# navigator8972/vae_assoc

Measured on AMD Instinct MI355X. Metric: paired-samples/sec (img+jnt assoc-VAE train step), higher is better.
Workload: dtype bf16

## Files before the change

### vae_assoc_amd/csrc/avae_device.h

```cpp
#pragma once
#include <hip/hip_runtime.h>
#include <math.h>
#include <stdint.h>
#include "../../include/avae.h"

namespace avae {

constexpr int kMaxMod = 4;
constexpr int kThreads = 256;
constexpr int kTileBytesK = 128;
constexpr int kRowAlign = 256;
constexpr int kLatentRows = 16;
constexpr int kAdamRows = 16;
constexpr int kCostHist = 4096;
constexpr int kSumsqThreads = 256;
constexpr int kSumsqMaxBlocks = 256;
constexpr int kSumsqQuads = 8;
inline int sumsq_blocks(long long p_int) {
    const long long quads = p_int / 4, per_block = (long long)kSumsqThreads * kSumsqQuads;
    const long long g = (quads + per_block - 1) / per_block;
    return (int)(g < 1 ? 1 : g > kSumsqMaxBlocks ? kSumsqMaxBlocks : g);
}
inline int sumsq_chain(long long p_int) {
    const long long quads = p_int / 4, per_pass = (long long)kSumsqThreads * sumsq_blocks(p_int);
// ... 20 lines not shown
    int lda, ldb;
    int tiles_m, tiles_n;
    int act;
    int ld0, ld1, ldx;
    int nz;
    int binary;
    int ksplit, kchunk;
    int bias_row;
    int bias_ep;
    int kin;
    int tile_off, tile_cnt;
    int slot_base;
    int n_slots;
    int n_mod;
    int bump_step;
    float scale;
    float lambda;
    float inv_bg;
    const void* A;
    const void* B;
    void* out0;
    void* out1;
    void* out2;
    const void* aux0;
    const void* aux1;
    const void* aux2;
    float* partial;
    const float* eps;
    float wts[kMaxMod];
    const void* tail_w;
    void* tail_out;
    const void* tail_aux;
    int tail_mode;
    int tail_n;
    int tail_ldw, tail_ldo, tail_ldx;
    int tail_act;
    int tail_kt;
    int conv;
    const unsigned char* present;
    int present_ld;
};

struct ConvA {
    const void* src;
    const void* consts;
    int M, K;
    int OHW, OW, IH, IW, Cin;
    int k, so, d, pad;
    int src_sb, src_sp;
    int ones;
    unsigned mg_ohw, mg_ow, mg_k, mg_cin;
};
constexpr int kMaxConvA = 12;
constexpr int kMaxItemsPerLaunch = 12;
constexpr int kMaxPf = 4;
struct LaunchArgs {
    int n_items;
    int grid_x;
    int sched;
    int n_pf;
    const void* pf_ptr[4];
    int pf_lines[4];
    const ConvA* conv_tab;
    WorkItem items[kMaxItemsPerLaunch];
};

struct TnItem {
    const void* A;
    const void* B;
    float* out;
    int M, N, K;
    int lda, ldb, ld0;
    int tiles_m, tiles_n;
    int ksplit, kchunk;
    int bias_row;
    int tile_off, tile_cnt;
    int conv;
    void* W; void* Wt;
    int ldw, ldt;
};
constexpr int kMaxTnItems = 32;
constexpr int kTnPieces = 8;
struct TnPiece { unsigned short item, tile_off, cum_end, pad; };
struct DevState;
struct TnLaunchArgs {
    int n_items;
    int grid_x;
    int xcd_group;
    int sched;
    int adam;
    long long d_theta, d_m, d_v;
    float beta1, beta2, eps;
    const DevState* st;
    const ConvA* conv_tab;
    int xcd_pieces;
    TnPiece pieces[8][kTnPieces];
    TnItem items[kMaxTnItems];
};
static_assert(sizeof(TnLaunchArgs) <= 4096, "kernel arguments are passed by value: 4 KiB");

struct DevState {
    long long step;
    float last_cost;
    float lr_t;
    float cost_hist[kCostHist];
};

struct ClipState {
    float max_norm;
    int skip_nonfinite;
    long long n_skipped;
    float partial[kSumsqMaxBlocks];
    float norm_hist[kCostHist];
};

struct EmaState {
    float decay;
    int warmup;
    int pad[30];
};
static_assert(sizeof(EmaState) == 128, "the average is line-aligned behind its settings");

struct HyperEntry { float kl, lambda, lr, pad; };
constexpr int kHyperSets = 16;
struct SchedState {
    avae_schedule sched[3];
    float lambda0, lr0;
    HyperEntry tab[kHyperSets];
    float hist[kCostHist][3];
};

__host__ __device__ inline float schedule_value(const avae_schedule& s, long long t) {
#pragma clang fp contract(off)
    long long u = t - 1;
    if (u < 0) u = 0;
    if (s.kind == AVAE_SCHED_PIECEWISE) {
        if (s.period > 0) u %= s.period;
        const int last = s.n_knots - 1;
        if (u <= s.knot_step[0]) return s.knot_value[0];
        if (u >= s.knot_step[last]) return s.knot_value[last];
        int i = 0;
        while (i + 1 < last && u >= s.knot_step[i + 1]) ++i;
        const double v0 = (double)s.knot_value[i], v1 = (double)s.knot_value[i + 1];
        const double f = (double)(u - s.knot_step[i]) / (double)(s.knot_step[i + 1] - s.knot_step[i]);
        return (float)(v0 + (v1 - v0) * f);
    }
    if (s.kind == AVAE_SCHED_EXP) {
        const double e = s.staircase ? (double)(u / s.decay_steps) : (double)u / (double)s.decay_steps;
        return (float)pow((double)s.decay_rate, e);
    }
    return 1.0f;
}

struct AdamItem {
    float* theta;
    float* m;
    float* v;
    const float* g;
    void* W;
    void* Wt;
    int rows, cols;
    int ld, ldt;
    int tiles_r, tiles_c, tile_base;
    int ldw;
    void* Wadj; void* Wf;
    int ldadj, ldf, adj_k, adj_cin;
};

constexpr int kMaxAdamItems = 80;
struct AdamArgs {
    const AdamItem* items;
    int n_items;
    int base[kMaxAdamItems];
    int mode;
    int book;
    float lr, beta1, beta2, eps;
    DevState* st;
    const float* cost_src;
    ClipState* clip;
    int n_partial;
    const EmaState* ema;
    float* avg;
// ... 155 lines not shown
    long long row0;
    unsigned long long seed; unsigned draw;
    const unsigned char* present; int pres_ld;
};
void launch_iw_latent(int compute_dtype, const IwLatentArgs& a, hipStream_t s);
struct IwRowsArgs {
    const float* xhat[kMaxMod]; int ldh[kMaxMod];
    const float* x[kMaxMod]; long long ldx[kMaxMod];
    int n_in[kMaxMod], binary[kMaxMod];
    float* ell;
    int n_dec, kc, n_mod;
    const unsigned char* present;
};
void launch_iw_rows(const IwRowsArgs& a, hipStream_t s);
struct IwReduceArgs {
    const float* ell; const float* r;
    float* state;
    float* out; int width;
    int rows, kc, src, n_mod;
    int first, last;
    float log_k;
    const unsigned char* present;
};
void launch_iw_reduce(const IwReduceArgs& a, hipStream_t s);

struct ImputeFuseArgs {
    const float* mulv[kMaxMod];
    unsigned mods;
    const unsigned char* present;
    float* fused;
    float* mu; float* lv;
    float* z32;
    void* Z[kMaxMod]; int ldz[kMaxMod]; int n_zdst;
    int rows, nz, n_mod;
};
void launch_impute_fuse(int compute_dtype, const ImputeFuseArgs& a, hipStream_t s);
struct ImputeAccumArgs {
    const float* xhat[kMaxMod]; int ldh[kMaxMod];
    float* mean[kMaxMod]; float* var[kMaxMod];
    int n_in[kMaxMod];
    int tile0[kMaxMod + 1];
    int col0[kMaxMod];
    float* state; int ld_state;
    int rows, kc, k0, K, n_mod;
};
void launch_impute_accum(const ImputeAccumArgs& a, hipStream_t s);

constexpr int kMaxWorld = 8;
constexpr int kIpcThreads = 256;
struct IpcArgs {
    float* g;
    long long off, granules;
    long long cost_idx;
    int world, rank, wire_bf16, blocks;
    unsigned char* peer[kMaxWorld];
    long long off_flag1, off_flag2;
    long long off_cost;
    long long off_seq;
    long long off_err;
    long long off_slots, slot_stride, off_res;
    unsigned long long timeout_ticks;
};
void launch_ipc_allreduce(const IpcArgs& a, hipStream_t s);
void launch_wire_pack(const float* g, void* wire, long long n, hipStream_t s);
void launch_wire_unpack(float* g, const void* wire, long long n, hipStream_t s);

struct LaunchEvents { hipEvent_t start, stop; };
extern thread_local LaunchEvents t_launch_events;

constexpr int kStampLaunches = 32, kStampBlocks = 1024, kStampWords = 8;

int tile_lds_bytes(int tile_cfg, bool two_c_tiles);
void launch_grouped(int compute_dtype, int tile_cfg, const LaunchArgs& args, int grid_x, int grid_y, int lds_bytes,
                    DevState* st, hipStream_t s, unsigned long long* stamps = nullptr, int launch_id = 0);
void launch_grouped_tn(int compute_dtype, int tile_cfg, const TnLaunchArgs& args, int grid_x, int grid_y, int lds_bytes,
                       DevState* st, hipStream_t s, unsigned long long* stamps = nullptr, int launch_id = 0);
void launch_adam(int compute_dtype, const AdamArgs& a, int n_blocks, hipStream_t s);
void launch_grad_sumsq(const float* g, long long p_int, float* partial, hipStream_t s);
void launch_prep(int compute_dtype, const PrepArgs& a, hipStream_t s);
const void* prep_kernel(int compute_dtype, bool masked, bool noisy, bool sched);
void launch_fill(void* base, int elem_bytes, unsigned bits, long long start, long long stride, int count, hipStream_t s);
void launch_sums(const ReduceArgs& a, int n_blocks, hipStream_t s);
int small_head_lds_bytes();
void launch_small_latb(int compute_dtype, int act, const LaunchArgs& args, int grid_x, int grid_y, int lds_bytes, DevState* st, hipStream_t s,
                       unsigned long long* stamps, int launch_id);
void launch_small_head(int compute_dtype, int act, const LaunchArgs& args, int grid_x, int grid_y, int lds_bytes, hipStream_t s,
                       unsigned long long* stamps, int launch_id);
void launch_small_tn(int compute_dtype, const TnLaunchArgs& args, int grid_x, int grid_y, hipStream_t s, unsigned long long* stamps, int launch_id);
void launch_small_loss(int compute_dtype, const LaunchArgs& args, int grid_x, int grid_y, int lds_bytes, hipStream_t s, unsigned long long* stamps, int launch_id);
void launch_small(int compute_dtype, const LaunchArgs& args, int grid_x, int grid_y, int lds_bytes, hipStream_t s, unsigned long long* stamps, int launch_id);
void launch_reduce(const ReduceArgs& a, int n_blocks, hipStream_t s);
void launch_chain2(int compute_dtype, const LaunchArgs& args, int grid_x, int grid_y, int lds_bytes, unsigned* counters, unsigned* err, hipStream_t s);

}
```

### vae_assoc_amd/csrc/avae_host.hip

```cpp
#include "avae_device.h"
#include "avae_complete.h"
#include "avae_retrieve.h"
#include "avae_latent_stats.h"
#include "../../include/avae.h"

#include <dlfcn.h>
#include <sched.h>
#include <unistd.h>

#include <algorithm>
#include <cctype>
#include <cstddef>
#include <cmath>
#include <cstdio>
#include <cstdlib>
#include <cstring>
#include <functional>
#include <map>
#include <mutex>
#include <stdexcept>
#include <string>
#include <vector>

using namespace avae;
// ... 110 lines not shown
    std::vector<ConvStage> cenc, cdec;
};

struct Launch {
    std::string name;
    int type = 0;
    int cfg = 0, first = 0, count = 0, blocks = 0, lds = 0;
    int lean_act = 0;
    int grid_x = 1, grid_y = 1;
    bool tn = false;
    LaunchArgs args{};
    TnLaunchArgs targs{};
    GatherArgs ga{};
    Col2imArgs ca{};
    ReduceArgs ra{};
    ThinArgs ta{};
    WadjArgs wa{};
    GpermArgs gp{};
    RowsumArgs rs{};
};

struct TimingRec { hipEvent_t a, b; int launch_name; };

struct StepGraph {
    hipGraphExec_t exec = nullptr;
    hipGraph_t graph = nullptr;
    hipGraphNode_t prep = nullptr;
    void release() {
        if (exec) (void)hipGraphExecDestroy(exec);
        if (graph) (void)hipGraphDestroy(graph);
        *this = StepGraph();
    }
};

struct StepPlan {
    std::vector<Launch> fwd;
    StepGraph full, multi[2], eval;
    void release() { full.release(); multi[0].release(); multi[1].release(); eval.release(); }
};

struct DevBuf {
    void* p = nullptr;
    size_t bytes = 0;
    DevBuf() = default;
    DevBuf(const DevBuf&) = delete;
    DevBuf& operator=(const DevBuf&) = delete;
    ~DevBuf() { if (p) (void)hipFree(p); }
    void* ensure(size_t n, bool zero = false) {
        if (p && n != bytes) throw Err("internal error: device scratch of " + std::to_string(bytes) + " bytes asked for as " + std::to_string(n));
        if (p) return p;
        void* q = nullptr;
        HIP_OK(hipMalloc(&q, n));
        if (zero && hipMemset(q, 0, n) != hipSuccess) { (void)hipFree(q); throw Err("hipMemset of fresh device scratch failed"); }
        p = q; bytes = n;
        return p;
    }
    template <typename T> T* as() const { return static_cast<T*>(p); }
};

}

struct avae_handle {
    avae_config cfg{};
    std::mutex mu;
    std::string err;
    int es = 2, KU = 64;
    int B = 0, Bp = 0, ldB = 0;
    int nz = 0, M = 0, ld_eps = 0;
    std::vector<Mod> mods;
    size_t P_flat = 0, P_int = 0, P_enc = 0;
    size_t off_theta = 0, off_m = 0, off_v = 0, off_g = 0;
    size_t stage_lo = 0, stage_bytes = 0;
    size_t off_eps = 0, off_partial = 0, off_state = 0, off_items = 0, off_adam = 0, off_inf = 0, off_stamps = 0, off_latent = 0;
    int n_partial = 0;
    size_t ws_bytes = 0;
    unsigned char* ws = nullptr;
    bool own_ws = false;
    hipStream_t cap_stream = nullptr;

    std::vector<WorkItem> items;
    std::vector<Launch> bwd;
    std::vector<Launch> wgrad;
    std::vector<Launch> wgrad_adam;
    int n_buckets = 1;
    int bwd_split = 0;
    std::vector<Launch> wgrad_b[2];
    struct Range { size_t off, count; };
    std::vector<Range> ranges_b[2];
    int adam_first_b[2] = {0, 0}, adam_count_b[2] = {0, 0}, adam_blocks_b[2] = {0, 0};
    std::vector<AdamItem> adam_items_b;
    size_t off_adam_b = 0;
    void* comm = nullptr;
    int comm_world = 1, comm_rank = 0;
    bool comm_on = false;
    size_t off_wire = 0;
    unsigned char* ipc_block = nullptr;
    size_t ipc_bytes = 0;
    unsigned char* ipc_peer[kMaxWorld] = {nullptr, nullptr, nullptr, nullptr, nullptr, nullptr, nullptr, nullptr};
    bool ipc_opened[kMaxWorld] = {false, false, false, false, false, false, false, false};
    bool ipc_attached = false;
    IpcArgs ipc_args{};
    hipStream_t comm_stream = nullptr;
    hipEvent_t ev_grad[2] = {nullptr, nullptr}, ev_red[2] = {nullptr, nullptr};
    std::vector<StepGraph> g_dp[2];
    StepGraph g_dpm[2];
    bool dp_graph_failed = false;
    Launch cost_only;
    std::vector<AdamItem> adam_items;
    int adam_blocks = 0;
    struct Inf { std::vector<WorkItem> items; std::vector<Launch> launches; int rows = -1; size_t dev_off = 0; };
    std::vector<Inf> inf_enc, inf_dec;
    struct Serve { int bucket = 0; std::vector<WorkItem> items; std::vector<Launch> launches; hipGraphExec_t graph = nullptr; ServeArgs in;
                   Launch in_launch; bool fused_in = false;
                   ServeInArgs in_lean; int in_lean_grid = 0; bool lean_in = false; };
    std::vector<Serve> serve;
    size_t off_slot = 0;
    DevBuf iw_buf;
    DevBuf imp_buf;
    DevBuf row_pres;
    DevBuf topk_buf;
    DevBuf stats_buf;
    size_t off_chain = 0;
    size_t off_consts = 0, off_conv_tab = 0;
    std::vector<ConvA> conv_tab;

    StepPlan plain, masked;
    DevBuf pres_buf;
    size_t pres_set = 0;

    avae_corruption corr{};
    unsigned drop_thr[kMaxMod] = {};

    bool clip_on = false;
    DevBuf clip_buf;
    long long clip_steps = 0;

    bool sched_on = false;
    DevBuf sched_buf;
    long long sched_steps = 0;

    bool ema_on = false, averaged = false;
    float ema_decay = 0.0f;
    int ema_warmup = 0;
    DevBuf ema_buf;

    struct Complete { bool built = false; std::vector<WorkItem> items; std::vector<Launch> fwd, bwd; CompleteArgs args{};
                      StepGraph g[3]; DevBuf buf; };
    Complete cmpl;

    hipStream_t last_stream = nullptr;
    bool has_last_stream = false;
    hipEvent_t ev_switch = nullptr;
    unsigned draw_id = 0;
    bool timing = false;
    bool debug_sync = false;
    std::vector<std::string> tnames;
    std::vector<TimingRec> trecs;

    template <typename T> T* at(size_t off) const { return reinterpret_cast<T*>(ws + off); }
    DevState* state() const { return at<DevState>(off_state); }
    float* grad() const { return at<float>(off_g); }
    float* ema_avg() const { return reinterpret_cast<float*>(ema_buf.as<unsigned char>() + sizeof(EmaState)); }
};

namespace {

inline int spread_ld(int ld, int KU, int es) {
    static const bool off = std::getenv("AVAE_NO_LD_SPREAD") != nullptr;
    return (!off && ((size_t)ld * es) % 512 == 0) ? ld + KU : ld;
}

Act make_act(Bump& b, int width, bool ones, int rows, int KU, int es, int ld = 0) {
    Act a;
    a.width = width;
    a.rows = rows;
    a.ones = ones;
    a.ld = ld > 0 ? ld : spread_ld((int)rup(width + 1, KU), KU, es);
    a.rm = b.take(rup(rows, kRowAlign) * (size_t)a.ld * es);
    return a;
}

Dense make_dense(Bump& b, size_t& pint, int in, int out, int KU, int es, bool head) {
    Dense d;
    d.in = in; d.out = out; d.head = head;
    d.ld = (int)rup(out, 32);
    d.ldw = spread_ld((int)rup(out, KU), KU, es);
    d.ldt = spread_ld((int)rup(in + 1, KU), KU, es);
    d.master = pint;
    pint += (size_t)(in + 1) * d.ld;
    d.W = b.take(rup(in + 1, kRowAlign) * (size_t)d.ldw * es);
    d.Wt = b.take(rup(out, kRowAlign) * (size_t)d.ldt * es);
    return d;
}

void check_config(const avae_config& c) {
    if (c.abi_version != AVAE_ABI_VERSION) throw Err("avae_config.abi_version mismatch");
    if (c.n_modalities < 1 || c.n_modalities > AVAE_MAX_MODALITIES) throw Err("n_modalities out of range");
    if (c.n_z < 1 || c.n_z > 64) throw Err("n_z must be in [1,64] (the fused head/latent epilogue holds 2*n_z columns in one tile)");
    if (c.batch_size < 1) throw Err("batch_size must be positive");
    if (c.compute_dtype != AVAE_F32 && c.compute_dtype != AVAE_BF16) throw Err("compute_dtype must be AVAE_F32 or AVAE_BF16");
    if (c.activation < AVAE_ACT_IDENTITY || c.activation > AVAE_ACT_TANH) throw Err("unknown activation");
    if (c.comm_buckets != 0 && c.comm_buckets != 1 && c.comm_buckets != 2) throw Err("comm_buckets must be 0, 1 or 2");
    if (c.wire_dtype != AVAE_F32 && c.wire_dtype != AVAE_BF16) throw Err("wire_dtype must be AVAE_F32 or AVAE_BF16");
    if (c.use_comm < AVAE_COMM_NONE || c.use_comm > AVAE_COMM_IPC) throw Err("use_comm must be AVAE_COMM_NONE, AVAE_COMM_RCCL or AVAE_COMM_IPC");
    for (int m = 0; m < c.n_modalities; ++m) {
        const avae_modality& mo = c.mod[m];
        if (mo.n_input < 1) throw Err("n_input must be positive");
        if (mo.hidden_conv) {
            if (mo.n_input != 784) throw Err("hidden_conv needs n_input = 784 (28x28 images)");
            if (!mo.binary) throw Err("hidden_conv needs a binary modality (the reference's non-binary conv decoder is shape-broken, vae_assoc.py:299)");
            if (mo.n_hidden_layers != 2 || mo.conv_gener[0] < 2 || mo.conv_gener[1] < 1) throw Err("hidden_conv needs n_hidden_recog_1/2 and n_hidden_gener_1 (>=2) / n_hidden_gener_2");
        }
        if (mo.n_hidden_layers < 1 || mo.n_hidden_layers > AVAE_MAX_HIDDEN) throw Err("n_hidden_layers out of range");
        for (int k = 0; k < mo.n_hidden_layers; ++k)
            if (mo.n_hidden[k] < 1) throw Err("hidden width must be positive");
    }
}

inline bool thin_fast(const ConvGeom& g) { return thin_fast_geometry(g) && !std::getenv("AVAE_NO_THIN_FAST"); }
inline int thin_split(const ConvGeom& g, int mode) {
    if (!thin_fast(g)) return kThinSplit;
    int sp[3] = {1, 4, 1};
    if (const char* e = std::getenv("AVAE_THIN_FAST_SPLIT")) std::sscanf(e, "%d,%d,%d", &sp[0], &sp[1], &sp[2]);
    const int v = sp[mode];
    return v == 1 || v == 2 || v == 4 ? v : 1;
}

void plan_memory(avae_handle* h) {
    const avae_config& c = h->cfg;
    h->es = c.compute_dtype == AVAE_BF16 ? 2 : 4;
    h->KU = kTileBytesK / h->es;
    h->B = c.batch_size;
    h->Bp = (int)rup(h->B, kRowAlign);
    h->ldB = (int)rup(h->B, h->KU);
    h->nz = c.n_z;
    h->ld_eps = (int)rup(c.n_z, 4);
    h->M = c.n_modalities;
    const int KU = h->KU, es = h->es, Bp = h->Bp, ldB = h->ldB, nz = h->nz, B = h->B;
// ... 638 lines not shown
    L.tn = true;
    for (int i = first; i < first + count; ++i) L.tn = L.tn && items[i].kind == K_WGRAD;
    if (count > (L.tn ? kMaxTnItems : kMaxItemsPerLaunch)) throw Err("internal error: too many items in one launch");
    std::memset(&L.args, 0, sizeof(L.args));
    std::memset(&L.targs, 0, sizeof(L.targs));
    if (L.tn) {
        int G = 1;
        if (L.cfg == 2) for (int g : {4, 2}) if (count % g == 0) { G = g; break; }
        if (const char* e = std::getenv("AVAE_TN_G")) G = std::atoi(e);
        if (G != 1 && G != 2 && G != 4 && G != 8) throw Err("AVAE_TN_G must be 1, 2, 4 or 8");
        auto tiles_of = [&](const WorkItem& w) { return w.tiles_m * w.tiles_n * (w.ksplit > 1 ? w.ksplit : 1); };
        int SX = L.grid_x;
        if (G == 1 && !std::getenv("AVAE_NO_TN_SLICES")) {
            long best = -1;
            for (int sx = 8; sx <= L.grid_x; sx += 8) {
                long entries = 0;
                for (int i = first; i < first + count; ++i) entries += (tiles_of(items[i]) + sx - 1) / sx;
                if (entries > kMaxTnItems) continue;
                if (best < 0 || entries * sx <= best) { best = entries * sx; SX = sx; }
            }
        }
        int n = 0;
        for (int i = 0; i < count; ++i) {
            const WorkItem& w = items[first + i];
            const int nt = tiles_of(w);
            for (int off = 0; off < nt; off += SX) {
                if (n >= kMaxTnItems) throw Err("internal error: too many weight-gradient entries");
                TnItem& t = L.targs.items[n++];
                t.A = w.A; t.B = w.B; t.out = reinterpret_cast<float*>(w.ksplit > 1 ? w.out1 : w.out0);
                t.bias_row = std::max(w.bias_row, 0);
                t.M = w.bias_row > 0 ? w.M - 1 : w.M; t.N = w.N; t.K = w.K; t.lda = w.lda; t.ldb = w.ldb; t.ld0 = w.ld0;
                t.tiles_m = w.tiles_m; t.tiles_n = w.tiles_n; t.ksplit = w.ksplit; t.kchunk = w.kchunk;
                t.tile_off = off; t.tile_cnt = std::min(SX, nt - off); t.conv = w.conv;
            }
        }
        if (G > 1 && !std::getenv("AVAE_NO_TN_BALANCE")) {
            std::vector<TnItem> ent(L.targs.items, L.targs.items + n);
            std::stable_sort(ent.begin(), ent.end(), [](const TnItem& a, const TnItem& b) { return a.tile_cnt > b.tile_cnt; });
            auto pack = [&](int g, std::vector<std::vector<TnItem>>& bins) {
                bins.assign(g, {});
                std::vector<long> load(g, 0);
                const int cap = kMaxTnItems / g;
                for (const TnItem& e : ent) {
                    int best = -1;
                    for (int p = 0; p < g; ++p) if ((int)bins[p].size() < cap && (best < 0 || load[p] < load[best])) best = p;
                    bins[best].push_back(e); load[best] += e.tile_cnt;
                }
                const long per_xcd = (*std::max_element(load.begin(), load.end()) * g + 7) / 8;
                return (per_xcd + 31) / 32;
            };
            std::vector<std::vector<TnItem>> bins, bins2;
            if (!std::getenv("AVAE_TN_G") && G == 4 && n * 2 <= kMaxTnItems * 2) {
                const long r4 = pack(4, bins), r2 = pack(2, bins2);
                if (r2 < r4) { G = 2; bins.swap(bins2); }
            } else {
                pack(G, bins);
            }
            size_t groups = 0;
            for (const auto& bn : bins) groups = std::max(groups, bn.size());
            std::memset(L.targs.items, 0, sizeof(L.targs.items));
            for (size_t g = 0; g < groups; ++g)
                for (int p = 0; p < G; ++p) if (g < bins[p].size()) L.targs.items[g * G + p] = bins[p][g];
            n = (int)groups * G;
        }
        L.grid_x = SX;
        L.targs.n_items = n;
        L.targs.grid_x = L.grid_x;
        L.targs.xcd_group = G;
        L.grid_y = (n + G - 1) / G * G;
        L.blocks = L.grid_x * L.grid_y;
    } else {
        L.args.n_items = count;
        L.args.grid_x = L.grid_x;
        for (int i = 0; i < count; ++i) L.args.items[i] = items[first + i];
    }
    L.args.conv_tab = L.targs.conv_tab = h->at<ConvA>(h->off_conv_tab);
    if (const char* e = std::getenv("AVAE_SCHED")) L.args.sched = L.targs.sched = std::atoi(e);
    if (*next_slot > h->n_partial) throw Err("internal error: cost partial slots overflow");
    return L;
}

void dp_ranges(const avae_handle* h, int* n_buckets, std::vector<avae_handle::Range> (&out)[2]);

void xcd_pieces(Launch& L) {
    TnLaunchArgs& a = L.targs;
    std::vector<TnItem> layers;
    for (int i = 0; i < a.n_items; ++i) {
        const TnItem& e = a.items[i];
        if (e.tile_cnt <= 0) continue;
        bool seen = false;
        for (const TnItem& l : layers) seen = seen || l.out == e.out;
        if (seen) continue;
        TnItem l = e;
        l.tile_off = 0; l.tile_cnt = e.tiles_m * e.tiles_n;
        if (l.tile_cnt > 65535) return;
        layers.push_back(l);
    }
    long total = 0;
    for (const TnItem& l : layers) total += l.tile_cnt;
    if (layers.empty() || total > 8L * 65535) return;
    const int quota = (int)((total + 7) / 8);
    std::vector<int> order(layers.size());
    for (size_t i = 0; i < order.size(); ++i) order[i] = (int)i;
    std::stable_sort(order.begin(), order.end(), [&](int x, int y) { return layers[x].tile_cnt > layers[y].tile_cnt; });
    struct Bin { int load = 0; std::vector<TnPiece> pc; };
    Bin bins[8];
    for (int li : order) {
        int off = 0, left = layers[li].tile_cnt;
        while (left > 0) {
            int best = -1;
            for (int b = 0; b < 8; ++b)
                if ((int)bins[b].pc.size() < kTnPieces && bins[b].load + left <= quota && (best < 0 || bins[b].load > bins[best].load)) best = b;
            int take = left;
            if (best < 0) {
                for (int b = 0; b < 8; ++b)
                    if ((int)bins[b].pc.size() < kTnPieces && bins[b].load < quota && (best < 0 || bins[b].load < bins[best].load)) best = b;
                if (best < 0) return;
                take = std::min(left, quota - bins[best].load);
            }
            bins[best].load += take;
            bins[best].pc.push_back(TnPiece{(unsigned short)li, (unsigned short)off, (unsigned short)bins[best].load, 0});
            off += take; left -= take;
        }
    }
    int longest = 0;
    for (int b = 0; b < 8; ++b) {
        longest = std::max(longest, bins[b].load);
        for (int i = 0; i < kTnPieces; ++i)
            a.pieces[b][i] = i < (int)bins[b].pc.size() ? bins[b].pc[i] : TnPiece{0, 0, (unsigned short)bins[b].load, 0};
    }
    std::memset(a.items, 0, sizeof(a.items));
    for (size_t i = 0; i < layers.size(); ++i) a.items[i] = layers[i];
    a.n_items = (int)layers.size();
    a.xcd_pieces = 1;
    L.grid_x = 8 * longest; L.grid_y = 1; L.blocks = L.grid_x;
    a.grid_x = L.grid_x;
}

struct Groups {
    avae_handle* h;
    std::vector<WorkItem>& items;
    int slot = 0;
    template <typename Fill> void operator()(const std::string& name, std::vector<Launch>& dst, Fill&& fill) {
        const int first = (int)items.size();
        fill();
        const int count = (int)items.size() - first;
        if (count > 0) dst.push_back(finish_launch(h, items, first, count, name, &slot));
    }
};

void build_training_plan(avae_handle* h) {
    h->items.clear(); h->plain.fwd.clear(); h->bwd.clear(); h->wgrad.clear(); h->conv_tab.clear();
    Builder bd(h, h->items, h->B, true);
    Groups group{h, h->items};
    int Lmax = 0;
    for (const Mod& md : h->mods) Lmax = std::max(Lmax, md.L);
    auto fuse_tail = [&](std::vector<Launch>& ls, int mode) {
        if (ls.size() < 2 || std::getenv("AVAE_NO_TAIL")) return false;
        Launch& Lp = ls[ls.size() - 2];
        Launch& Lc = ls[ls.size() - 1];
        if (Lp.type != 0 || Lc.type != 0 || Lp.tn || Lc.tn || Lp.cfg != 3) return false;
        const int want_p = mode == 1 ? K_FWD_HEAD : K_DGRAD_LATENT, want_c = mode == 1 ? K_FWD_HIDDEN : K_DGRAD_HIDDEN;
        std::vector<int> prod(Lc.count, -1);
        for (int i = 0; i < Lc.count; ++i) {
            const WorkItem& c = h->items[Lc.first + i];
            if (c.kind != want_c || c.bias_ep || c.K > 2 * h->KU || c.N > 1024) return false;
            for (int k = 0; k < Lp.count; ++k) {
                const WorkItem& n = h->items[Lp.first + k];
                if (n.kind != want_p || n.M != c.M) continue;
                const void* res = mode == 1 ? n.out1 : n.out0;
                const int ldres = mode == 1 ? n.ld1 : n.ld0;
                if (res && res == c.A && ldres == c.lda) prod[i] = k;
            }
            if (prod[i] < 0) return false;
        }
        for (int i = 0; i < Lc.count; ++i) {
            const WorkItem c = h->items[Lc.first + i];
            for (WorkItem* n : {&h->items[Lp.first + prod[i]], &Lp.args.items[prod[i]]}) {
                n->tail_mode = mode; n->tail_w = c.B; n->tail_ldw = c.ldb; n->tail_n = c.N; n->tail_out = c.out0; n->tail_ldo = c.ld0;
                n->tail_aux = c.aux0; n->tail_ldx = c.ldx; n->tail_act = c.act; n->tail_kt = c.K / h->KU;
                n->tiles_n = (c.N + 63) / 64;
            }
        }
        int max_tiles = 1;
        for (int k = 0; k < Lp.count; ++k) max_tiles = std::max(max_tiles, h->items[Lp.first + k].tiles_m * h->items[Lp.first + k].tiles_n);
        Lp.grid_x = (max_tiles + 7) & ~7; Lp.blocks = Lp.grid_x * Lp.grid_y; Lp.args.grid_x = Lp.grid_x;
        Lp.name += "+" + Lc.name;
        ls.pop_back();
        if (!std::getenv("AVAE_NO_LEAN") && !std::getenv("AVAE_NO_LEAN_HEAD")) {
            bool lean = true;
            int act = -1;
            for (int k = 0; k < Lp.count; ++k) {
                const WorkItem& n = h->items[Lp.first + k];
                if (n.kind == K_COST) continue;
                lean = lean && n.kind == want_p && n.tail_mode == mode
                            && (act < 0 || act == n.tail_act) && n.K > 0 && 2 * n.nz <= 64 && n.tail_kt >= 1 && n.tail_kt <= 2;
                act = n.tail_act;
            }
            if (lean && mode == 1)
                for (int k = 0; k < Lp.count; ++k) lean = lean && h->items[Lp.first + k].kind == K_FWD_HEAD && h->items[Lp.first + k].out1 != nullptr;
            if (lean) { Lp.cfg = mode == 2 ? 10 : 11; Lp.lds = small_head_lds_bytes(); Lp.lean_act = act; }
        }
        return true;
    };
    auto every_conv = [](const Mod&) { return true; };
    auto gather_launch = [&](const std::string& name, std::vector<Launch>& dst, auto&& stage_of, auto&& src_of, auto&& want) {
        Launch L;
        L.name = name; L.type = 1;
        int base = 0;
        for (Mod& md : h->mods) if (md.conv && want(md)) {
            GatherSeg g = bd.gather_seg(stage_of(md), src_of(md));
            g.tile_base = base; base += g.tiles_r * g.tiles_c;
            L.ga.seg[L.ga.n_seg++] = g;
        }
        L.blocks = base;
        if (base > 0) dst.push_back(L);
    };
    auto col2im_launch = [&](const std::string& name, std::vector<Launch>& dst, auto&& stage_of, auto&& prev_of, auto&& want) {
        Launch L;
        L.name = name; L.type = 2;
        int base = 0;
        for (Mod& md : h->mods) if (md.conv && want(md)) {
            Col2imSeg c = bd.col2im_seg(stage_of(md), prev_of(md), md);
            c.tile_base = base; base += c.tiles_r * c.tiles_c;
            L.ca.seg[L.ca.n_seg++] = c;
        }
        L.blocks = base;
        if (base > 0) dst.push_back(L);
    };
    auto thin_launch = [&](const std::string& name, std::vector<Launch>& dst, int mode, int i) {
        Launch L;
        L.name = name; L.type = 4;
        L.ta.mode = mode;
        int base = 0;
        for (Mod& md : h->mods) if (md.conv && md.cdec[i].thin) {
            ThinSeg t = bd.thin_seg(md.cdec[i], md.cdec[i - 1]);
            t.split = thin_split(md.cdec[i].g, mode);
            t.block_base = base;
            base += h->B * t.split;
            L.ta.seg[L.ta.n_seg++] = t;
        }
        L.blocks = base;
        if (base > 0) dst.push_back(L);
    };
    auto is_adj = [&](int i) { bool t = false; for (const Mod& md : h->mods) t = t || (md.conv && i >= 0 && i <= 3 && md.cdec[i].adj); return t; };
    auto is_thin = [&](int i) { bool t = false; for (const Mod& md : h->mods) t = t || (md.conv && md.cdec[i].thin); return t; };
    bool any_conv = false;
    for (const Mod& md : h->mods) any_conv = any_conv || md.conv;
    for (int k = 0; k < Lmax; ++k)
        group("fwd_enc" + std::to_string(k + 1), h->plain.fwd, [&] {
            for (Mod& md : h->mods) if (k < md.L) h->items.push_back(bd.fwd_hidden(k == 0 ? md.X0 : md.E[k - 1], md.enc[k], md.E[k]));
        });
    if (std::getenv("AVAE_CHAIN2") && !any_conv && h->plain.fwd.size() == 2 && h->plain.fwd[0].cfg == 7 && h->plain.fwd[1].cfg == 7 && h->plain.fwd[0].count == h->plain.fwd[1].count
        && 2 * h->plain.fwd[0].count <= kMaxItemsPerLaunch) {
        Launch& A = h->plain.fwd[0];
        const Launch& Bn = h->plain.fwd[1];
        bool ok = true;
        for (int i = 0; i < A.count; ++i) {
            const WorkItem& a = A.args.items[i];
            const WorkItem& c = Bn.args.items[i];
            ok = ok && a.kind == K_FWD_HIDDEN && c.kind == K_FWD_HIDDEN && a.act == c.act && a.M == c.M && a.N == c.N && a.tiles_m == c.tiles_m && a.tiles_n == c.tiles_n
                    && c.A == a.out0 && c.lda == a.ld0 && a.N % 4 == 0 && a.tiles_m <= 64;
        }
        if (ok) {
            for (int i = 0; i < A.count; ++i) A.args.items[A.count + i] = Bn.args.items[i];
            A.args.n_items = 2 * A.count;
            A.cfg = 13; A.name += "+" + Bn.name;
            h->plain.fwd.pop_back();
        }
    }
    if (any_conv) {
        for (int i = 0; i < 3; ++i) {
            auto src_of = [&, i](Mod& md) { return i == 0 ? h->at<void>(md.X0.rm) : h->at<void>(md.cenc[i - 1].Y.rm); };
            gather_launch("conv_enc" + std::to_string(i + 1) + "_im2col", h->plain.fwd, [&](Mod& md) -> const ConvStage& { return md.cenc[i]; },
                          src_of, [i](const Mod& md) { return !md.cenc[i].impl; });
            group("conv_enc" + std::to_string(i + 1), h->plain.fwd, [&] {
                for (Mod& md : h->mods) if (md.conv) h->items.push_back(md.cenc[i].impl ? bd.conv_fwd_impl(md.cenc[i], src_of(md)) : bd.conv_fwd(md.cenc[i])); });
        }
        gather_launch("conv_head_im2col", h->plain.fwd, [&](Mod& md) -> const ConvStage& { return md.cenc[3]; },
                      [&](Mod& md) { return h->at<void>(md.cenc[2].Y.rm); }, [](const Mod& md) { return !md.cenc[3].impl; });
    }
    group("fwd_head", h->plain.fwd, [&] { for (Mod& md : h->mods) h->items.push_back(bd.fwd_head(md, true, md.conv && md.cenc[3].impl)); });
    bool latent_alone = false;
    {
// ... 307 lines not shown
                for (int k = md.L - 1; k >= 1; --k) set[0].push_back(bd.wgrad(md.D[k - 1], md.dec[k], md.dD[k]));
                set[0].push_back(bd.wgrad(md.Z, md.dec[0], md.dD[0]));
                set[1].push_back(bd.wgrad(md.E.back(), md.head, md.dH));
                for (int k = md.L - 1; k >= 1; --k) set[1].push_back(bd.wgrad(md.E[k - 1], md.enc[k], md.dE[k]));
                set[1].push_back(bd.wgrad(md.X0, md.enc[0], md.dE[0]));
            }
            wgrad_launches(set[0], h->wgrad_b[0], "wgrad_dec");
            wgrad_launches(set[1], h->wgrad_b[1], "wgrad_enc");
        }
        for (int i = 1; i <= 3; ++i) if (is_thin(i)) thin_launch("conv_dec" + std::to_string(i + 1) + "_wgrad_direct", h->wgrad, 2, i);
        {
            Launch L;
            L.name = "conv_bias_rowsum"; L.type = 8;
            int base = 0;
            for (Mod& md : h->mods) if (md.conv) for (const ConvStage& st : md.cdec) if (st.adj && !st.impl_w) {
                RowsumSeg& g = L.rs.seg[L.rs.n_seg++];
                g.src = h->at<void>(st.dY.rm); g.part = h->at<float>(st.rs_part); g.ld = st.dY.ld;
                g.rows = h->B * st.g.OH * st.g.OW; g.cols = st.d.out; g.cols4 = st.rs_cols4; g.n_blocks = kRowsumBlocks;
                g.cpow = 4; while (g.cpow < g.cols4) g.cpow *= 2;
                if (g.cpow > 64) throw Err("internal error: bias row sums hold at most 64 columns");
                g.block_base = base; base += kRowsumBlocks;
            }
            L.blocks = base;
            if (base > 0) h->wgrad.push_back(L);
        }
        {
            Launch R;
            R.name = "conv_wgrad_sums"; R.type = 5;
            int base = 0;
            for (Mod& md : h->mods) if (md.conv) for (const ConvStage& st : md.cdec) if (st.adj && !st.impl_w) {
                ReduceSeg& g = R.ra.seg[R.ra.n_seg++];
                g.dst = h->grad() + st.d.master + (size_t)st.d.in * st.d.ld; g.src = h->at<float>(st.rs_part);
                g.n = st.d.out; g.parts = kRowsumBlocks; g.stride = st.rs_cols4; g.dst_ld = 1;
                g.block_base = base; base += (g.n + 3) / 4;
            }
            for (Mod& md : h->mods) if (md.conv) for (const ConvStage& st : md.cdec) if (st.thin) {
                ReduceSeg& g = R.ra.seg[R.ra.n_seg++];
                g.dst = h->grad() + st.d.master; g.src = h->at<float>(st.thin_part);
                g.n = st.d.in + 1; g.parts = st.thin_blocks; g.stride = st.thin_kp; g.dst_ld = st.d.ld;
                g.block_base = base; base += (g.n + 3) / 4;
            }
            R.blocks = base;
            for (int i = 0; i < R.ra.n_seg; ++i) { R.ra.seg[i].colsum = 1; R.ra.seg[i].perm_k = 0; }
            if (base > 0) h->wgrad.push_back(R);
        }
        {
            Launch R;
            R.name = "wgrad_reduce"; R.type = 3;
            int base = 0;
            Launch* prev = (!h->wgrad.empty() && h->wgrad.back().type == 5 && !std::getenv("AVAE_NO_SUMS_MERGE")) ? &h->wgrad.back() : nullptr;
            if (prev) { R = *prev; R.name = prev->name + "+wgrad_reduce"; R.type = 9; base = prev->blocks; }
            for (const WorkItem& w : wg) if (w.ksplit > 1) {
                if (R.ra.n_seg >= kMaxReduceSegs) throw Err("internal error: too many split weight gradients");
                ReduceSeg& g = R.ra.seg[R.ra.n_seg++];
                g.dst = reinterpret_cast<float*>(w.out0); g.src = reinterpret_cast<const float*>(w.out1);
                g.n = w.M * w.ld0; g.parts = w.ksplit; g.stride = (long long)w.M * w.ld0;
                g.colsum = 0; g.perm_k = 0;
                if (!std::getenv("AVAE_NO_SUMS_MERGE"))
                    for (Mod& md : h->mods) if (md.conv) for (const ConvStage& st : md.cdec) if (st.adj && st.aksplit > 1 && g.dst == h->at<float>(st.Gadj)) {
                        g.dst = h->grad() + st.d.master;
                        g.perm_k = st.g.k; g.perm_cin = st.g.Cin; g.perm_cout = st.d.out; g.perm_ldga = st.ldga; g.perm_ld = st.d.ld;
                    }
                g.block_base = base; base += (g.n / 4 + kThreads - 1) / kThreads;
            }
            R.blocks = base;
            if (prev && base > prev->blocks) *prev = R;
            else if (!prev && base > 0) h->wgrad.push_back(R);
        }
        {
            Launch L;
            L.name = "conv_wgrad_perm"; L.type = 7;
            int base = 0;
            for (Mod& md : h->mods) if (md.conv) for (const ConvStage& st : md.cdec) if (st.adj && !st.impl_w) {
                if (st.aksplit > 1 && !std::getenv("AVAE_NO_SUMS_MERGE")) continue;
                GpermSeg& g = L.gp.seg[L.gp.n_seg++];
                g.Gadj = h->at<float>(st.Gadj); g.G = h->grad() + st.d.master; g.ldga = st.ldga; g.ld = st.d.ld;
                g.k = st.g.k; g.Cin = st.g.Cin; g.Cout = st.d.out;
                g.block_base = base; base += (st.g.Cin * st.g.k * st.g.k * st.d.out + kThreads - 1) / kThreads;
            }
            L.blocks = base;
            if (base > 0) h->wgrad.push_back(L);
        }
    }
    h->wgrad_adam.clear();
    if (!any_conv && h->wgrad.size() == 1 && h->wgrad[0].tn && h->wgrad[0].cfg == 0 && h->wgrad[0].targs.xcd_group == 1
        && !std::getenv("AVAE_NO_LEAN") && !std::getenv("AVAE_NO_ADAM_FUSE")) {
        Launch L = h->wgrad[0];
        bool ok = true;
        for (int i = 0; i < L.targs.n_items && ok; ++i) {
            TnItem& t = L.targs.items[i];
            ok = t.ksplit <= 1 && t.bias_row == 0 && t.K > 0;
            const Dense* dm = nullptr;
            for (const Mod& md : h->mods) {
                auto look = [&](const Dense& d) { if (h->grad() + d.master == t.out) dm = &d; };
                for (const Dense& d : md.enc) look(d);
                look(md.head);
                for (const Dense& d : md.dec) look(d);
                look(md.outl);
            }
            ok = ok && dm && t.M == dm->in + 1 && t.N == dm->out && t.ld0 == dm->ld;
            if (ok) { t.W = h->at<void>(dm->W); t.Wt = h->at<void>(dm->Wt); t.ldw = dm->ldw; t.ldt = dm->ldt; }
        }
        if (ok) {
            L.cfg = 12; L.name = "wgrad+adam";
            L.targs.adam = 1;
            L.targs.d_theta = h->at<float>(h->off_theta) - h->grad();
            L.targs.d_m = h->at<float>(h->off_m) - h->grad();
            L.targs.d_v = h->at<float>(h->off_v) - h->grad();
            L.targs.beta1 = h->cfg.beta1; L.targs.beta2 = h->cfg.beta2; L.targs.eps = h->cfg.adam_eps;
            L.targs.st = h->state();
            if (!std::getenv("AVAE_NO_XCD_PIECES")) xcd_pieces(L);
            h->wgrad_adam.push_back(L);
        }
    }
    if (!std::getenv("AVAE_NO_WARM")) {
        std::vector<Launch*> seq;
        for (Launch& L : h->plain.fwd) seq.push_back(&L);
        for (Launch& L : h->bwd) seq.push_back(&L);
        for (size_t i = 0; i < seq.size(); ++i) {
            Launch& L = *seq[i];
            if (L.type != 0 || L.tn || (L.cfg != 2 && L.cfg != 6)) continue;
            for (size_t j = i + 1; j < seq.size(); ++j) {
                const Launch& Nx = *seq[j];
                if (Nx.type != 0) continue;
                if (Nx.tn) break;
                for (int k = 0; k < Nx.args.n_items && L.args.n_pf < kMaxPf; ++k) {
                    const WorkItem& w = Nx.args.items[k];
                    if (!is_gemm(w.kind) || w.kind == K_WGRAD) continue;
                    const long bytes = (long)w.N * w.ldb * h->es;
                    if (bytes < 128 * 1024) continue;
                    L.args.pf_ptr[L.args.n_pf] = w.B; L.args.pf_lines[L.args.n_pf] = (int)(bytes / 128); ++L.args.n_pf;
                }
                break;
            }
        }
    }
    {
        const int first = (int)h->items.size();
        h->items.push_back(bd.cost(false));
        h->cost_only = finish_launch(h, h->items, first, 1, "cost_reduce", &group.slot);
    }

    h->adam_items.clear();
    int base = 0;
    auto add = [&](const Dense& d) {
        AdamItem a;
        std::memset(&a, 0, sizeof(a));
        a.theta = h->at<float>(h->off_theta) + d.master;
        a.m = h->at<float>(h->off_m) + d.master;
        a.v = h->at<float>(h->off_v) + d.master;
        a.g = h->grad() + d.master;
        a.W = h->at<void>(d.W); a.Wt = h->at<void>(d.Wt);
        a.rows = d.in + 1; a.cols = d.out; a.ld = d.ld; a.ldw = d.ldw; a.ldt = d.ldt;
        a.tiles_r = (a.rows + kAdamRows - 1) / kAdamRows; a.tiles_c = (a.cols + 63) / 64; a.tile_base = base;
        base += a.tiles_r * a.tiles_c;
        h->adam_items.push_back(a);
    };
    for (const Mod& md : h->mods) {
        if (md.conv) {
            for (const std::vector<ConvStage>* side : {&md.cenc, &md.cdec})
                for (const ConvStage& st : *side) {
                    add(st.d);
                    if ((st.adj && !std::getenv("AVAE_NO_WADJ_FOLD")) || st.impl_bwd) {
                        AdamItem& a = h->adam_items.back();
                        a.Wadj = h->at<void>(st.Wadj); a.ldadj = st.ldadj; a.adj_k = st.g.k; a.adj_cin = st.g.Cin;
                        if (st.adj) { a.Wf = h->at<void>(st.Wf); a.ldf = st.ldf; }
                    }
                }
            continue;
        }
        for (const Dense& d : md.enc) add(d);
        add(md.head);
        for (const Dense& d : md.dec) add(d);
        add(md.outl);
    }
    h->adam_blocks = base;
    h->adam_items_b.clear();
    for (int bk = 0; bk < 2; ++bk) {
        h->adam_first_b[bk] = (int)h->adam_items_b.size();
        int tb = 0;
        size_t i = 0;
        for (const Mod& md : h->mods) {
            const size_t n_enc = md.conv ? md.cenc.size() : (size_t)md.L + 1, n_all = md.conv ? md.cenc.size() + md.cdec.size() : 2 * (size_t)md.L + 2;
            for (size_t k = 0; k < n_all; ++k) {
                const int which = h->n_buckets == 1 ? 0 : (k < n_enc ? 1 : 0);
                if (which == bk) {
                    AdamItem a = h->adam_items[i + k];
                    a.tile_base = tb; tb += a.tiles_r * a.tiles_c;
                    h->adam_items_b.push_back(a);
                }
            }
            i += n_all;
        }
        h->adam_count_b[bk] = (int)h->adam_items_b.size() - h->adam_first_b[bk];
        h->adam_blocks_b[bk] = tb;
// ... 21 lines not shown
        inf.launches.push_back(L);
    };
    if (enc && md.conv) {
        for (int i = 0; i < 3; ++i) {
            gather1(md.cenc[i], i == 0 ? h->at<void>(md.X0.rm) : h->at<void>(md.cenc[i - 1].Y.rm), "inf_conv_im2col");
            one(bd.conv_fwd(md.cenc[i]), "inf_conv_enc");
        }
        gather1(md.cenc[3], h->at<void>(md.cenc[2].Y.rm), "inf_conv_im2col");
        one(bd.fwd_head(md, true), "inf_head");
    } else if (enc) {
        for (int k = 0; k < md.L; ++k) one(bd.fwd_hidden(k == 0 ? md.X0 : md.E[k - 1], md.enc[k], md.E[k]), "inf_enc");
        one(bd.fwd_head(md, true), "inf_head");
    } else if (md.conv) {
        for (int i = 0; i < 4; ++i) {
            if (md.cdec[i].dense_map) {
                Launch L;
                L.name = "inf_conv_dec_direct"; L.type = 4;
                L.ta.mode = 0;
                ThinSeg t = bd.thin_seg(md.cdec[i], md.cdec[i - 1]);
                t.block_base = 0;
                L.ta.seg[0] = t; L.ta.n_seg = 1;
                L.blocks = rows * t.split;
                inf.launches.push_back(L);
                continue;
            }
            gather1(md.cdec[i], i == 0 ? h->at<void>(md.Z.rm) : h->at<void>(md.cdec[i - 1].Y.rm), "inf_conv_im2col");
            one(bd.conv_fwd(md.cdec[i]), "inf_conv_dec");
        }
        if (!md.cdec[3].dense_map) gather1(md.cdec[4], h->at<void>(md.cdec[3].Y.rm), "inf_conv_im2col");
        one(bd.fwd_out(md, m, false), "inf_out");
    } else {
        for (int k = 0; k < md.L; ++k) one(bd.fwd_hidden(k == 0 ? md.Z : md.D[k - 1], md.dec[k], md.D[k]), "inf_dec");
        one(bd.fwd_out(md, m, false), "inf_out");
    }
    inf.rows = rows;
}

int tname_id(avae_handle* h, const std::string& n) {
    for (size_t i = 0; i < h->tnames.size(); ++i) if (h->tnames[i] == n) return (int)i;
    h->tnames.push_back(n);
    return (int)h->tnames.size() - 1;
}

struct Timed {
    avae_handle* h; hipStream_t s; bool on; hipEvent_t a = nullptr, b = nullptr; int id = 0;
    Timed(avae_handle* h_, hipStream_t s_, const std::string& name) : h(h_), s(s_), on(h_->timing && h_->trecs.size() < 200000) {
        if (!on) return;
        id = tname_id(h, name);
        HIP_OK(hipEventCreate(&a)); HIP_OK(hipEventCreate(&b));
        t_launch_events = LaunchEvents{a, b};
    }
    ~Timed() {
        if (!on) return;
        if (t_launch_events.start) {
            t_launch_events = LaunchEvents{nullptr, nullptr};
            (void)hipEventRecord(a, s); (void)hipEventRecord(b, s);
        }
        h->trecs.push_back(TimingRec{a, b, id});
    }
};

template <typename F> void timed_launch(avae_handle* h, hipStream_t s, const char* name, F&& launch) {
    Timed t(h, s, name);
    launch();
    LAUNCH_OK(name);
}

Launch relocated(const avae_handle* h, const Launch& L0, int j, const HyperEntry* hyper = nullptr) {
    Launch L = L0;
    const unsigned char* lo = h->ws + h->stage_lo;
    const unsigned char* hi = lo + h->stage_bytes;
    const size_t delta = (size_t)j * h->stage_bytes;
    auto fix = [&](auto& ptr) {
        const unsigned char* q = reinterpret_cast<const unsigned char*>(ptr);
        if (q >= lo && q < hi) ptr = reinterpret_cast<std::remove_reference_t<decltype(ptr)>>(const_cast<unsigned char*>(q) + delta);
    };
    for (int i = 0; i < L.args.n_items && L.type == 0; ++i) {
        WorkItem& w = L.args.items[i];
        fix(w.A); fix(w.B); fix(w.out0); fix(w.out1); fix(w.out2); fix(w.aux0); fix(w.aux1); fix(w.aux2); fix(w.eps);
        fix(w.tail_w); fix(w.tail_out); fix(w.tail_aux);
        if (w.present) w.present += (size_t)j * h->pres_set;
        if (hyper && (w.kind == K_LATENT || (w.kind == K_COST && w.bump_step))) w.tail_w = hyper + j;
    }
    for (int i = 0; i < L.targs.n_items && L.type == 0; ++i) { TnItem& t = L.targs.items[i]; fix(t.A); fix(t.B); fix(t.out); }
    for (int i = 0; i < L.ga.n_seg && L.type == 1; ++i) fix(L.ga.seg[i].src);
    return L;
}

void run_launch(avae_handle* h, const Launch& L, hipStream_t s, unsigned long long* stamps, int stamp) {
    Timed t(h, s, L.name);
    if (L.type == 1) launch_gather(h->cfg.compute_dtype, L.ga, L.blocks, s);
    else if (L.type == 2) launch_col2im(h->cfg.compute_dtype, L.ca, L.blocks, s);
    else if (L.type == 3) launch_reduce(L.ra, L.blocks, s);
    else if (L.type == 4) launch_thin(h->cfg.compute_dtype, L.ta, L.blocks, s);
    else if (L.type == 5) launch_colsum(L.ra, L.blocks, s);
    else if (L.type == 6) launch_wadj(h->cfg.compute_dtype, L.wa, L.blocks, s);
    else if (L.type == 7) launch_gperm(L.gp, L.blocks, s);
    else if (L.type == 8) launch_rowsum(h->cfg.compute_dtype, L.rs, L.blocks, s);
    else if (L.type == 9) launch_sums(L.ra, L.blocks, s);
    else if (L.cfg == 13) launch_chain2(h->cfg.compute_dtype, L.args, L.grid_x, L.grid_y, L.lds, h->at<unsigned>(h->off_chain), h->at<unsigned>(h->off_chain) + kMaxMod * 64, s);
    else if (L.cfg == 11) launch_small_head(h->cfg.compute_dtype, L.lean_act, L.args, L.grid_x, L.grid_y, L.lds, s, stamps, stamp);
    else if (L.cfg == 10) launch_small_latb(h->cfg.compute_dtype, L.lean_act, L.args, L.grid_x, L.grid_y, L.lds, h->state(), s, stamps, stamp);
    else if (L.cfg == 9) launch_small_loss(h->cfg.compute_dtype, L.args, L.grid_x, L.grid_y, L.lds, s, stamps, stamp);
    else if (L.cfg == 7) launch_small(h->cfg.compute_dtype, L.args, L.grid_x, L.grid_y, L.lds, s, stamps, stamp);
    else if (L.tn && L.cfg == 12) launch_small_tn(h->cfg.compute_dtype, L.targs, L.grid_x, L.grid_y, s, stamps, stamp);
    else if (L.tn) launch_grouped_tn(h->cfg.compute_dtype, L.cfg, L.targs, L.grid_x, L.grid_y, L.lds, h->state(), s, stamps, stamp);
    else launch_grouped(h->cfg.compute_dtype, L.cfg, L.args, L.grid_x, L.grid_y, L.lds, h->state(), s, stamps, stamp);
    LAUNCH_OK(L.name);
    if (h->debug_sync) {
        std::fprintf(stderr, "[avae] launch %s type=%d cfg=%d items=%d blocks=%d\n", L.name.c_str(), L.type, L.cfg, L.count, L.blocks);
        for (int i = 0; i < L.args.n_items && L.type == 0; ++i)
            std::fprintf(stderr, "        item kind=%d M=%d N=%d K=%d lda=%d ldb=%d tiles=%dx%d\n", L.args.items[i].kind, L.args.items[i].M,
                         L.args.items[i].N, L.args.items[i].K, L.args.items[i].lda, L.args.items[i].ldb, L.args.items[i].tiles_m, L.args.items[i].tiles_n);
        for (int i = 0; i < L.ga.n_seg && L.type == 1; ++i)
            std::fprintf(stderr, "        gather B=%d IH=%d Cin=%d OH=%d k=%d so=%d d=%d pad=%d sb=%d sp=%d ones=%d ldp=%d tiles=%dx%d\n", L.ga.seg[i].g.B, L.ga.seg[i].g.IH,
                         L.ga.seg[i].g.Cin, L.ga.seg[i].g.OH, L.ga.seg[i].g.k, L.ga.seg[i].g.so, L.ga.seg[i].g.d, L.ga.seg[i].g.pad, L.ga.seg[i].g.src_sb, L.ga.seg[i].g.src_sp,
                         L.ga.seg[i].g.ones, L.ga.seg[i].ldp, L.ga.seg[i].tiles_r, L.ga.seg[i].tiles_c);
        for (int i = 0; i < L.ca.n_seg && L.type == 2; ++i)
            std::fprintf(stderr, "        col2im B=%d IH=%d Cin=%d OH=%d k=%d lddp=%d lda=%d g0=%p tiles=%dx%d\n", L.ca.seg[i].g.B, L.ca.seg[i].g.IH, L.ca.seg[i].g.Cin,
                         L.ca.seg[i].g.OH, L.ca.seg[i].g.k, L.ca.seg[i].lddp, L.ca.seg[i].lda, (const void*)L.ca.seg[i].g0, L.ca.seg[i].tiles_r, L.ca.seg[i].tiles_c);
        std::fflush(stderr);
        HIP_OK(hipStreamSynchronize(s));
    }
}

bool has_hyper_item(const Launch& L) {
    for (int i = 0; i < L.args.n_items && L.type == 0; ++i)
        if (L.args.items[i].kind == K_LATENT || (L.args.items[i].kind == K_COST && L.args.items[i].bump_step)) return true;
    return false;
}

void run_set(avae_handle* h, const std::vector<Launch>& ls, size_t lo, size_t hi, int j, hipStream_t s, int stamp_base = -1, bool train = false) {
    unsigned long long* stamps = nullptr;
#ifdef AVAE_STAMPS
    if (stamp_base >= 0) stamps = h->at<unsigned long long>(h->off_stamps);
#endif
    const HyperEntry* hyper = nullptr;
    if (train && h->sched_on) {
        if (!h->sched_buf.p) throw Err("internal error: a schedule is on without its device state");
        if (j < 0 || j >= kHyperSets) throw Err("internal error: staging set outside the schedule table");
        hyper = h->sched_buf.as<SchedState>()->tab;
    }
    for (size_t i = lo; i < hi && i < ls.size(); ++i) {
        const int k = stamp_base + (int)(i - lo);
        if (j == 0 && !(hyper && has_hyper_item(ls[i]))) run_launch(h, ls[i], s, stamps, k);
        else run_launch(h, relocated(h, ls[i], j, hyper), s, stamps, k);
    }
}

void run_launches(avae_handle* h, const std::vector<Launch>& ls, hipStream_t s) { run_set(h, ls, 0, ls.size(), 0, s); }

void run_adam(avae_handle* h, int mode, hipStream_t s, int bucket = -1, bool from_avg = false) {
    AdamArgs a;
    std::memset(&a, 0, sizeof(a));
    int blocks = h->adam_blocks;
    if (bucket < 0) {
        a.items = h->at<AdamItem>(h->off_adam);
        a.n_items = (int)h->adam_items.size();
        if (a.n_items > kMaxAdamItems) throw Err("internal error: too many Adam items");
        for (int i = 0; i < a.n_items; ++i) a.base[i] = h->adam_items[i].tile_base;
    } else {
        a.items = h->at<AdamItem>(h->off_adam_b) + h->adam_first_b[bucket];
        a.n_items = h->adam_count_b[bucket];
        for (int i = 0; i < a.n_items; ++i) a.base[i] = h->adam_items_b[h->adam_first_b[bucket] + i].tile_base;
        blocks = h->adam_blocks_b[bucket];
        if (blocks == 0) return;
    }
    a.book = (bucket <= 0) ? 1 : 0;
    a.mode = mode;
    a.lr = h->cfg.learning_rate; a.beta1 = h->cfg.beta1; a.beta2 = h->cfg.beta2; a.eps = h->cfg.adam_eps;
    a.st = h->state();
    a.cost_src = h->grad() + h->P_int;
    a.clip = (mode == 0 && h->clip_on) ? h->clip_buf.as<ClipState>() : nullptr;
    a.n_partial = sumsq_blocks((long long)h->P_int);
    if (mode == 0 ? h->ema_on : from_avg) {
        if (!h->ema_buf.p) throw Err("internal error: averaging is on without its device state");
        a.ema = h->ema_buf.as<EmaState>(); a.avg = h->ema_avg(); a.theta0 = h->at<float>(h->off_theta);
    }
    Timed t(h, s, mode == 0 ? (bucket < 0 ? "adam" : bucket == 0 ? "adam_dec" : "adam_enc") : "shadow_refresh");
    launch_adam(h->cfg.compute_dtype, a, blocks, s);
    LAUNCH_OK(mode == 0 ? "adam" : "shadow_refresh");
}

void run_grad_sumsq(avae_handle* h, hipStream_t s) {
    ClipState* cs = h->clip_buf.as<ClipState>();
    if (!cs) throw Err("internal error: clipping is on without its device state");
    timed_launch(h, s, "grad_sumsq", [&] { launch_grad_sumsq(h->grad(), (long long)h->P_int, cs->partial, s); });
}

struct PrepIn { const float* const* in = nullptr; const int32_t* in_ld = nullptr; bool corrupt = false; };

PrepArgs new_prep(const avae_handle* h, unsigned long long salt, int row0 = 0) {
    PrepArgs a;
// ... 36 lines not shown
    fill_prep_eps(h, a, eps, rows);
    a.n_steps = n_steps; a.blocks_per_step = a.total_tiles + a.eps_blocks; a.set_stride = (long long)h->stage_bytes;
    if (present) { a.pres_src = present; a.pres_dst = h->pres_buf.as<unsigned char>(); a.pres_ld = h->M; }
    if (h->sched_on && salt == kTrainSalt) a.sched = h->sched_buf.as<SchedState>();
    return a;
}

void run_prep_batch(avae_handle* h, const float* const* x, const int32_t* x_ld, const float* eps, int rows,
                    unsigned long long salt, hipStream_t s, const uint8_t* present = nullptr, int n_steps = 1, const PrepIn& pin = PrepIn()) {
    const PrepArgs a = make_prep_batch(h, x, x_ld, eps, rows, salt, n_steps, present, pin);
    timed_launch(h, s, "prep", [&] { launch_prep(h->cfg.compute_dtype, a, s); });
}

struct PrepOne {
    const float* src; int src_ld, rows, cols;
    const Act& dst;
    int row0;
    PrepOne(const float* src_, int src_ld_, int rows_, int cols_, const Act& dst_, int row0_ = 0)
        : src(src_), src_ld(src_ld_), rows(rows_), cols(cols_), dst(dst_), row0(row0_) {}
    float* dst32 = nullptr; int ld32 = 0;
    bool eps = false;
    const float* eps_src = nullptr;
    unsigned long long salt = 0;
    PrepOne& with_eps(const float* e, unsigned long long salt_ = 0) { eps = true; eps_src = e; salt = salt_; return *this; }
    const unsigned char* pres_src = nullptr; unsigned char* pres_dst = nullptr; int pres_ld = 0;
};

void run_prep_single(avae_handle* h, const PrepOne& p, hipStream_t s) {
    PrepArgs a = new_prep(h, p.salt, p.row0);
    if (p.pres_src) { a.pres_src = p.pres_src; a.pres_dst = p.pres_dst; a.pres_ld = p.pres_ld; }
    if (p.src || p.pres_src) {
        a.n_seg = 1;
        a.total_tiles = fill_prep_seg(h, a.seg[0], p.src, p.src_ld, p.rows, p.cols, p.dst, p.dst32, p.ld32, 0);
    }
    if (p.eps) fill_prep_eps(h, a, p.eps_src, p.rows);
    launch_prep(h->cfg.compute_dtype, a, s);
    LAUNCH_OK("prep");
}

StepGraph capture(avae_handle* h, const std::function<void(hipStream_t)>& body, bool with_prep = false) {
    StepGraph sg;
    const bool tsave = h->timing;
    h->timing = false;
    HIP_OK(hipStreamBeginCapture(h->cap_stream, hipStreamCaptureModeThreadLocal));
    try { body(h->cap_stream); }
    catch (...) { (void)hipStreamEndCapture(h->cap_stream, &sg.graph); sg.release(); h->timing = tsave; throw; }
    h->timing = tsave;
    HIP_OK(hipStreamEndCapture(h->cap_stream, &sg.graph));
    try {
        if (with_prep) {
            size_t n_root = 0;
            HIP_OK(hipGraphGetRootNodes(sg.graph, nullptr, &n_root));
            if (n_root != 1) throw Err("internal error: the captured step is not a chain");
            HIP_OK(hipGraphGetRootNodes(sg.graph, &sg.prep, &n_root));
            hipGraphNodeType ty;
            HIP_OK(hipGraphNodeGetType(sg.prep, &ty));
            if (ty != hipGraphNodeTypeKernel) throw Err("internal error: the captured step does not start with the staging kernel");
        }
        HIP_OK(hipGraphInstantiate(&sg.exec, sg.graph, nullptr, nullptr, 0));
        if (!with_prep) { HIP_OK(hipGraphDestroy(sg.graph)); sg.graph = nullptr; }
    } catch (...) { sg.release(); throw; }
    return sg;
}

void patch_prep(avae_handle* h, const StepGraph& sg, const float* const* x, const int32_t* x_ld, const float* eps,
                int n_steps, const uint8_t* present, const PrepIn& pin) {
    PrepArgs a = make_prep_batch(h, x, x_ld, eps, h->B, kTrainSalt, n_steps, present, pin);
    void* kp[1] = {&a};
    hipKernelNodeParams np;
    std::memset(&np, 0, sizeof(np));
    np.func = const_cast<void*>(prep_kernel(h->cfg.compute_dtype, present != nullptr, a.noisy != 0, a.sched != nullptr));
    np.gridDim = dim3((a.total_tiles + a.eps_blocks) * n_steps); np.blockDim = dim3(kThreads);
    np.sharedMemBytes = 0; np.kernelParams = kp; np.extra = nullptr;
    HIP_OK(hipGraphExecKernelNodeSetParams(sg.exec, sg.prep, &np));
}

void fill_ones(avae_handle* h, const Act& a, hipStream_t s) {
    if (!a.ones) return;
    const unsigned bits = h->es == 2 ? 0x3F80u : 0x3F800000u;
    launch_fill(h->at<void>(a.rm), h->es, bits, a.width, a.ld, h->B, s);
    LAUNCH_OK("fill");
}

void step_body(avae_handle* h, const std::vector<Launch>& fwd, hipStream_t s, int j, int stamp_base = -1) {
    auto sb = [&](size_t k) { return stamp_base < 0 ? -1 : stamp_base + (int)k; };
    run_set(h, fwd, 0, fwd.size(), j, s, stamp_base, true);
    run_set(h, h->bwd, 0, h->bwd.size(), j, s, sb(fwd.size()), true);
    if (!h->wgrad_adam.empty() && !h->clip_on && !h->ema_on) {
        run_set(h, h->wgrad_adam, 0, h->wgrad_adam.size(), j, s, sb(fwd.size() + h->bwd.size()), true);
        return;
    }
    run_set(h, h->wgrad, 0, h->wgrad.size(), j, s, sb(fwd.size() + h->bwd.size()), true);
    if (h->clip_on) run_grad_sumsq(h, s);
    run_adam(h, 0, s);
}

void capture_steps(avae_handle* h, StepPlan& p, const uint8_t* present) {
    std::vector<const float*> x0(h->M, h->at<float>(h->mods[0].X32));
    try {
        p.full = capture(h, [&](hipStream_t cs) {
            run_prep_batch(h, x0.data(), nullptr, nullptr, h->B, kTrainSalt, cs, present);
            step_body(h, p.fwd, cs, 0, 0);
        }, true);
        for (int gi = 0; gi < 2; ++gi) p.multi[gi] = capture(h, [&](hipStream_t cs) {
            run_prep_batch(h, x0.data(), nullptr, nullptr, h->B, kTrainSalt, cs, present, kMultiSizes[gi]);
            for (int j = 0; j < kMultiSizes[gi]; ++j) step_body(h, p.fwd, cs, j);
        }, true);
    } catch (...) { p.full.release(); p.multi[0].release(); p.multi[1].release(); throw; }
}

void capture_plan(avae_handle* h, StepPlan& p, const uint8_t* present) {
    try {
        capture_steps(h, p, present);
        p.eval = capture(h, [&](hipStream_t cs) { run_launches(h, p.fwd, cs); run_launch(h, h->cost_only, cs, nullptr, -1); });
    } catch (...) { p.release(); throw; }
}

void init_device(avae_handle* h) {
    hipStream_t s = h->cap_stream;
    HIP_OK(hipMemsetAsync(h->ws, 0, h->ws_bytes, s));
    for (const Mod& md : h->mods) {
        for (int j = 0; j < kMultiSteps; ++j) {
            Act x = md.X0;
            x.rm += (size_t)j * h->stage_bytes;
            fill_ones(h, x, s);
        }
        for (const Act& a : md.E) fill_ones(h, a, s);
        fill_ones(h, md.Z, s);
        for (const Act& a : md.D) fill_ones(h, a, s);
        if (md.conv && md.cdec[3].dense_map) fill_ones(h, md.cdec[3].Y, s);
    }
    build_training_plan(h);
    HIP_OK(hipMemcpyAsync(h->at<void>(h->off_adam), h->adam_items.data(), h->adam_items.size() * sizeof(AdamItem), hipMemcpyHostToDevice, s));
    HIP_OK(hipMemcpyAsync(h->at<void>(h->off_adam_b), h->adam_items_b.data(), h->adam_items_b.size() * sizeof(AdamItem), hipMemcpyHostToDevice, s));
    {
        static const unsigned char c32_bf16[32] = {0, 0, 0, 0, 0, 0, 0, 0, 0, 0, 0, 0, 0, 0, 0, 0, 0x80, 0x3F};
        static const unsigned char c32_f32[32] = {0, 0, 0, 0, 0, 0, 0, 0, 0, 0, 0, 0, 0, 0, 0, 0, 0, 0, 0x80, 0x3F};
        HIP_OK(hipMemcpyAsync(h->at<void>(h->off_consts), h->es == 2 ? c32_bf16 : c32_f32, 32, hipMemcpyHostToDevice, s));
        if (!h->conv_tab.empty()) {
            const unsigned char* lo = h->ws + h->stage_lo;
            for (const ConvA& c : h->conv_tab)
                if (reinterpret_cast<const unsigned char*>(c.src) >= lo && reinterpret_cast<const unsigned char*>(c.src) < lo + h->stage_bytes * kMultiSteps)
                    throw Err("internal error: an implicit patch matrix on a staged input (not relocatable per step)");
            HIP_OK(hipMemcpyAsync(h->at<void>(h->off_conv_tab), h->conv_tab.data(), h->conv_tab.size() * sizeof(ConvA), hipMemcpyHostToDevice, s));
        }
    }
    size_t off = h->off_inf;
    h->inf_enc.assign(h->M, avae_handle::Inf());
    h->inf_dec.assign(h->M, avae_handle::Inf());
    for (int m = 0; m < h->M; ++m) {
        h->inf_enc[m].dev_off = off; off += ((size_t)h->mods[m].L + 1) * sizeof(WorkItem);
        h->inf_dec[m].dev_off = off; off += ((size_t)h->mods[m].L + 1) * sizeof(WorkItem);
    }
    HIP_OK(hipStreamSynchronize(s));
    if (h->cfg.use_graph) capture_plan(h, h->plain, nullptr);
}

void comm_check_error(avae_handle* h);

void fetch_cost(avae_handle* h, float* cost_host, bool from_state, hipStream_t s) {
    if (!cost_host) return;
    const void* src = from_state ? (const void*)&h->state()->last_cost : (const void*)(h->grad() + h->P_int);
    HIP_OK(hipMemcpyAsync(cost_host, src, sizeof(float), hipMemcpyDeviceToHost, s));
    HIP_OK(hipStreamSynchronize(s));
    comm_check_error(h);
}

void copy_rows(void* dst, size_t dpitch, const void* src, size_t spitch, size_t width, size_t rows, hipStream_t s) {
    HIP_OK(hipMemcpy2DAsync(dst, dpitch, src, spitch, width, rows, hipMemcpyDeviceToDevice, s));
}

hipStream_t on_stream(avae_handle* h, void* stream) {
    hipStream_t s = reinterpret_cast<hipStream_t>(stream);
    if (h->has_last_stream && s != h->last_stream) {
        if (!h->ev_switch) HIP_OK(hipEventCreateWithFlags(&h->ev_switch, hipEventDisableTiming));
        if (hipEventRecord(h->ev_switch, h->last_stream) == hipSuccess) HIP_OK(hipStreamWaitEvent(s, h->ev_switch, 0));
        else (void)hipGetLastError();
    }
    h->last_stream = s; h->has_last_stream = true;
    return s;
}

void check_schedule(const avae_schedule& c, const std::string& who) {
    auto fail = [&](const std::string& what) { throw Err(who + ": " + what); };
    if (c.kind == AVAE_SCHED_NONE) return;
    if (c.kind == AVAE_SCHED_PIECEWISE) {
        if (c.n_knots < 1 || c.n_knots > AVAE_SCHED_MAX_KNOTS)
            fail("n_knots = " + std::to_string(c.n_knots) + " must be in [1, " + std::to_string(AVAE_SCHED_MAX_KNOTS) + "]");
        if (c.period < 0) fail("period = " + std::to_string((long long)c.period) + " must be >= 0");
// ... 734 lines not shown
    HIP_OK(hipDeviceSynchronize());
    run_adam(h, 1, nullptr, -1, on);
    HIP_OK(hipDeviceSynchronize());
    h->averaged = on;
}

void set_ema(avae_handle* h, float decay, int32_t warmup) {
    if (!(decay >= 0.0f && decay < 1.0f)) throw Err("avae_set_ema: decay must be in (0, 1), or 0 to switch averaging off");
    if (warmup != 0 && warmup != 1) throw Err("avae_set_ema: warmup must be 0 or 1");
    const bool on = decay > 0.0f;
    HIP_OK(hipDeviceSynchronize());
    if (!on && !h->ema_buf.p) return;
    if (!on && h->averaged) use_averaged(h, false);
    h->ema_buf.ensure(sizeof(EmaState) + h->P_int * sizeof(float));
    if (on) {
        EmaState v;
        std::memset(&v, 0, sizeof(v));
        v.decay = decay; v.warmup = warmup;
        HIP_OK(hipMemcpy(h->ema_buf.p, &v, sizeof(v), hipMemcpyHostToDevice));
        h->ema_decay = decay; h->ema_warmup = warmup;
    }
    if (on == h->ema_on && (!h->cfg.use_graph || h->plain.full.exec)) return;
    if (on && !h->ema_on) ema_from_theta(h);
    h->plain.full.release(); h->plain.multi[0].release(); h->plain.multi[1].release();
    h->masked.full.release(); h->masked.multi[0].release(); h->masked.multi[1].release();
    for (StepGraph& g : h->g_dpm) g.release();
    h->ema_on = on;
    if (h->cfg.use_graph) {
        capture_steps(h, h->plain, nullptr);
        if (!h->masked.fwd.empty()) capture_steps(h, h->masked, h->pres_buf.as<unsigned char>());
    }
}

void destroy_handle(avae_handle* h) {
    int prev_dev = -1;
    if (hipGetDevice(&prev_dev) != hipSuccess) prev_dev = -1;
    (void)hipSetDevice(h->cfg.device);
    (void)hipDeviceSynchronize();
    h->plain.release();
    h->masked.release();
    for (StepGraph& g : h->g_dpm) g.release();
    for (std::vector<StepGraph>& v : h->g_dp) for (StepGraph& g : v) g.release();
    for (avae_handle::Serve& sv : h->serve) if (sv.graph) (void)hipGraphExecDestroy(sv.graph);
    for (StepGraph& g : h->cmpl.g) g.release();
    if (h->ev_switch) (void)hipEventDestroy(h->ev_switch);
    if (h->comm) { try { (void)Rccl::get().destroy(h->comm); } catch (...) {} }
    for (int r = 0; r < kMaxWorld; ++r) if (h->ipc_opened[r] && h->ipc_peer[r]) (void)hipIpcCloseMemHandle(h->ipc_peer[r]);
    if (h->ipc_block) (void)hipFree(h->ipc_block);
    for (int b = 0; b < 2; ++b) { if (h->ev_grad[b]) (void)hipEventDestroy(h->ev_grad[b]); if (h->ev_red[b]) (void)hipEventDestroy(h->ev_red[b]); }
    if (h->comm_stream) (void)hipStreamDestroy(h->comm_stream);
    for (TimingRec& r : h->trecs) { (void)hipEventDestroy(r.a); (void)hipEventDestroy(r.b); }
    if (h->cap_stream) (void)hipStreamDestroy(h->cap_stream);
    if (h->own_ws && h->ws) (void)hipFree(h->ws);
    const int dev = h->cfg.device;
    delete h;
    if (prev_dev >= 0 && prev_dev != dev) (void)hipSetDevice(prev_dev);
}

}

extern "C" {

int avae_workspace_bytes(const avae_config* cfg, size_t* bytes) {
    try {
        if (!cfg || !bytes) throw Err("null argument");
        check_config(*cfg);
        avae_handle tmp;
        tmp.cfg = *cfg;
        plan_memory(&tmp);
        *bytes = tmp.ws_bytes;
        return 0;
    } catch (const std::exception& e) { g_create_error = e.what(); return 2; }
}

int avae_create(const avae_config* cfg, avae_handle** out) {
    avae_handle* h = nullptr;
    try {
        if (!cfg || !out) throw Err("null argument");
        check_config(*cfg);
        h = new avae_handle();
        h->cfg = *cfg;
        if (const char* e = std::getenv("AVAE_DEBUG_SYNC")) h->debug_sync = e[0] == '1';
        if (h->debug_sync) h->cfg.use_graph = 0;
        if (h->cfg.beta1 == 0.f && h->cfg.beta2 == 0.f && h->cfg.adam_eps == 0.f) { h->cfg.beta1 = 0.9f; h->cfg.beta2 = 0.999f; h->cfg.adam_eps = 1e-8f; }
        int ndev = 0;
        HIP_OK(hipGetDeviceCount(&ndev));
        if (ndev < 1) throw Err("no HIP device: libavae has no CPU fallback");
        if (h->cfg.device < 0 || h->cfg.device >= ndev) throw Err("device ordinal out of range");
        DeviceGuard dg(h->cfg.device);
        hipDeviceProp_t prop;
        HIP_OK(hipGetDeviceProperties(&prop, h->cfg.device));
        if (std::string(prop.gcnArchName).rfind("gfx950", 0) != 0)
            throw Err(std::string("libavae is built for gfx950 only; device is ") + prop.gcnArchName);
        plan_memory(h);
        if (cfg->workspace) {
            if (cfg->workspace_bytes < h->ws_bytes) throw Err("workspace too small");
            if (reinterpret_cast<uintptr_t>(cfg->workspace) % 256) throw Err("workspace must be 256-byte aligned");
            h->ws = reinterpret_cast<unsigned char*>(cfg->workspace);
        } else {
            HIP_OK(hipMalloc(reinterpret_cast<void**>(&h->ws), h->ws_bytes));
            h->own_ws = true;
        }
        HIP_OK(hipStreamCreateWithFlags(&h->cap_stream, hipStreamNonBlocking));
        init_device(h);
        if (h->cfg.use_comm) comm_init(h);
        *out = h;
        return 0;
    } catch (const std::exception& e) {
        g_create_error = e.what();
        if (h) destroy_handle(h);
        return 2;
    }
}

void avae_destroy(avae_handle* h) {
    if (h) destroy_handle(h);
}

const char* avae_last_error(const avae_handle* h) { return h ? h->err.c_str() : g_create_error.c_str(); }

int avae_param_count(const avae_handle* h, size_t* n) {
    if (!h || !n) return 1;
    *n = h->P_flat;
    return 0;
}

int avae_get_params(avae_handle* h, float* host_dst) {
    return guarded(h, [&] { std::vector<float> I; master_to_host(h, h->off_theta, I); convert_params<false>(h, host_dst, I.data()); });
}

int avae_set_params(avae_handle* h, const float* host_src) {
    return guarded(h, [&] {
        std::vector<float> I(h->P_int, 0.0f);
        convert_params<true>(h, const_cast<float*>(host_src), I.data());
        host_to_master(h, h->off_theta, I);
        run_adam(h, 1, nullptr);
        HIP_OK(hipDeviceSynchronize());
        h->averaged = false;
    });
}

int avae_get_grads(avae_handle* h, float* host_dst) {
    return guarded(h, [&] { std::vector<float> I; master_to_host(h, h->off_g, I); convert_params<false>(h, host_dst, I.data()); });
}

int avae_get_opt_state(avae_handle* h, float* host_m, float* host_v, int64_t* step) {
    return guarded(h, [&] {
        std::vector<float> I;
        if (host_m) { master_to_host(h, h->off_m, I); convert_params<false>(h, host_m, I.data()); }
        if (host_v) { master_to_host(h, h->off_v, I); convert_params<false>(h, host_v, I.data()); }
        if (step) { long long st = 0; HIP_OK(hipDeviceSynchronize()); HIP_OK(hipMemcpy(&st, &h->state()->step, sizeof(st), hipMemcpyDeviceToHost)); *step = st; }
    });
}

int avae_set_opt_state(avae_handle* h, const float* host_m, const float* host_v, int64_t step) {
    return guarded(h, [&] {
        std::vector<float> I(h->P_int, 0.0f);
        if (host_m) { convert_params<true>(h, const_cast<float*>(host_m), I.data()); host_to_master(h, h->off_m, I); }
        if (host_v) { std::fill(I.begin(), I.end(), 0.0f); convert_params<true>(h, const_cast<float*>(host_v), I.data()); host_to_master(h, h->off_v, I); }
        long long st = step;
        HIP_OK(hipDeviceSynchronize());
        HIP_OK(hipMemcpy(&h->state()->step, &st, sizeof(st), hipMemcpyHostToDevice));
    });
}

int avae_stage_batches_in(avae_handle* h, int32_t n_steps, const float* const* x_dev, const int32_t* x_ld, const float* const* in_dev,
// ... 860 lines not shown
            }
            uint64_t P = 0;
            if (std::fread(&P, 8, 1, f) != 1 || P != h->P_flat) throw Err("checkpoint parameter count mismatch");
            if (std::fread(&st, 8, 1, f) != 1) throw Err("truncated checkpoint");
            th.resize(P); mm.resize(P); vv.resize(P);
            if (std::fread(th.data(), 4, P, f) != P || std::fread(mm.data(), 4, P, f) != P || std::fread(vv.data(), 4, P, f) != P)
                throw Err("truncated checkpoint");
            if (version == 3) {
                if (std::fread(&decay, 4, 1, f) != 1) throw Err("truncated checkpoint");
                warmup = r32();
                if (!(decay > 0.0f && decay < 1.0f) || warmup > 1) throw Err("checkpoint holds invalid averaging settings");
                av.resize(P);
                if (std::fread(av.data(), 4, P, f) != P) throw Err("truncated checkpoint");
            }
        } catch (...) { std::fclose(f); throw; }
        std::fclose(f);
        std::vector<float> I(h->P_int, 0.0f);
        convert_params<true>(h, th.data(), I.data()); host_to_master(h, h->off_theta, I);
        std::fill(I.begin(), I.end(), 0.0f); convert_params<true>(h, mm.data(), I.data()); host_to_master(h, h->off_m, I);
        std::fill(I.begin(), I.end(), 0.0f); convert_params<true>(h, vv.data(), I.data()); host_to_master(h, h->off_v, I);
        long long step = st;
        HIP_OK(hipMemcpy(&h->state()->step, &step, sizeof(step), hipMemcpyHostToDevice));
        run_adam(h, 1, nullptr);
        HIP_OK(hipDeviceSynchronize());
        h->averaged = false;
        if (version == 3) {
            set_ema(h, decay, (int32_t)warmup);
            std::fill(I.begin(), I.end(), 0.0f); convert_params<true>(h, av.data(), I.data()); host_to_ema(h, I);
        } else if (h->ema_on) {
            ema_from_theta(h);
        }
    });
}

int avae_synchronize(avae_handle* h) {
    return guarded(h, [&] { HIP_OK(hipDeviceSynchronize()); comm_check_error(h); });
}

int avae_timing_enable(avae_handle* h, int32_t on) {
    return guarded(h, [&] {
        HIP_OK(hipDeviceSynchronize());
        for (TimingRec& r : h->trecs) { (void)hipEventDestroy(r.a); (void)hipEventDestroy(r.b); }
        h->trecs.clear();
        h->timing = on != 0;
    });
}

int avae_timing_report(avae_handle* h, char* buf, size_t buf_bytes) {
    return guarded(h, [&] {
        HIP_OK(hipDeviceSynchronize());
        const double cal_ms = 0.0;
        std::vector<double> sum(h->tnames.size(), 0.0), mn(h->tnames.size(), 1e30);
        std::vector<long> cnt(h->tnames.size(), 0);
        for (TimingRec& r : h->trecs) {
            float ms = 0.f;
            HIP_OK(hipEventElapsedTime(&ms, r.a, r.b));
            sum[r.launch_name] += ms; cnt[r.launch_name] += 1; mn[r.launch_name] = std::min(mn[r.launch_name], (double)ms);
        }
        std::string out;
        for (size_t i = 0; i < h->tnames.size(); ++i) {
            if (!cnt[i]) continue;
            char line[256];
            std::snprintf(line, sizeof(line), "%s %ld %.6f %.6f\n", h->tnames[i].c_str(), cnt[i], std::max(0.0, sum[i] / cnt[i] - cal_ms), std::max(0.0, mn[i] - cal_ms));
            out += line;
        }
        if (!buf || buf_bytes == 0) throw Err("null buffer");
        std::snprintf(buf, buf_bytes, "%s", out.c_str());
    });
}

int avae_comm_allreduce(avae_handle* h, int32_t bucket, void* stream) {
    return guarded(h, [&] {
        if (!h->comm_on) throw Err("avae_comm_allreduce: the replica has no library-owned collective (use_comm)");
        if (bucket < 0 || bucket >= h->n_buckets) throw Err("data-parallel bucket out of range");
        dp_allreduce(h, bucket, on_stream(h, stream));
    });
}

int avae_debug_fetch(avae_handle* h, const char* name, float* host_dst, size_t max_floats, size_t* n_floats) {
    return guarded(h, [&] {
        std::string n(name ? name : "");
        const void* src = nullptr;
        size_t cnt = 0;
        if (n == "eps") {
            cnt = (size_t)h->B * h->nz;
            if (cnt > max_floats) throw Err("debug_fetch: destination too small");
            HIP_OK(hipDeviceSynchronize());
            HIP_OK(hipMemcpy2D(host_dst, (size_t)h->nz * 4, h->at<void>(h->off_eps), (size_t)h->ld_eps * 4, (size_t)h->nz * 4, h->B, hipMemcpyDeviceToHost));
            if (n_floats) *n_floats = cnt;
            return;
        }
#ifdef AVAE_STAMPS
        else if (n == "stamps") { src = h->at<void>(h->off_stamps); cnt = (size_t)kStampLaunches * kStampBlocks * kStampWords * 2; }
#endif
        else if ((n[0] == 'E' || n[0] == 'D') && n.size() >= 4 && n.find('_') != std::string::npos) {
            const int m = std::atoi(n.c_str() + 1), k = std::atoi(n.c_str() + n.find('_') + 1);
            if (m < 0 || m >= h->M || h->mods[m].conv || k < 0 || k >= h->mods[m].L) throw Err("debug_fetch: no such hidden layer");
            const Act& a = n[0] == 'E' ? h->mods[m].E[k] : h->mods[m].D[k];
            cnt = (size_t)h->B * a.width;
            if (cnt > max_floats) throw Err("debug_fetch: destination too small");
            HIP_OK(hipDeviceSynchronize());
            std::vector<unsigned char> raw((size_t)h->B * a.ld * h->es);
            HIP_OK(hipMemcpy(raw.data(), h->at<void>(a.rm), raw.size(), hipMemcpyDeviceToHost));
            for (int r = 0; r < h->B; ++r)
                for (int c = 0; c < a.width; ++c) {
                    float v;
                    if (h->es == 2) { const uint32_t u = (uint32_t)reinterpret_cast<const uint16_t*>(raw.data())[(size_t)r * a.ld + c] << 16; std::memcpy(&v, &u, 4); }
                    else v = reinterpret_cast<const float*>(raw.data())[(size_t)r * a.ld + c];
                    host_dst[(size_t)r * a.width + c] = v;
                }
            if (n_floats) *n_floats = cnt;
            return;
        }
        else if ((n[0] == 'X' || n[0] == 'T') && n.size() >= 2 && std::isdigit((unsigned char)n[1])) {
            const int m = std::atoi(n.c_str() + 1);
            if (m < 0 || m >= h->M) throw Err("debug_fetch: modality out of range");
            const Mod& md = h->mods[m];
            const bool enc = n[0] == 'X';
            const int ld = enc ? md.X0.ld : md.ld32, esz = enc ? h->es : 4;
            cnt = (size_t)h->B * md.n_in;
            if (cnt > max_floats) throw Err("debug_fetch: destination too small");
            HIP_OK(hipDeviceSynchronize());
            std::vector<unsigned char> raw((size_t)h->B * ld * esz);
            HIP_OK(hipMemcpy(raw.data(), enc ? h->at<void>(md.X0.rm) : h->at<void>(md.X32), raw.size(), hipMemcpyDeviceToHost));
            for (int r = 0; r < h->B; ++r)
                for (int c = 0; c < md.n_in; ++c) {
                    float v;
                    if (esz == 2) { const uint32_t u = (uint32_t)reinterpret_cast<const uint16_t*>(raw.data())[(size_t)r * ld + c] << 16; std::memcpy(&v, &u, 4); }
                    else v = reinterpret_cast<const float*>(raw.data())[(size_t)r * ld + c];
                    host_dst[(size_t)r * md.n_in + c] = v;
                }
            if (n_floats) *n_floats = cnt;
            return;
        }
        else if (n == "shadow_err") {
            if (max_floats < 4) throw Err("debug_fetch: destination too small");
            HIP_OK(hipDeviceSynchronize());
            auto round_ct = [&](float v) {
                if (h->es == 4) return v;
                uint32_t u; std::memcpy(&u, &v, 4);
                if ((u & 0x7fffffffu) > 0x7f800000u) return v;
                u += 0x7fffu + ((u >> 16) & 1u); u &= 0xffff0000u;
                float r; std::memcpy(&r, &u, 4); return r;
            };
            auto elem = [&](const std::vector<unsigned char>& raw, size_t i) {
                float v;
                if (h->es == 2) { const uint32_t u = (uint32_t)reinterpret_cast<const uint16_t*>(raw.data())[i] << 16; std::memcpy(&v, &u, 4); }
                else v = reinterpret_cast<const float*>(raw.data())[i];
                return v;
            };
            float ew = 0.f, et = 0.f;
            int cnt = 0, worst = -1;
            auto check = [&](const Dense& d) {
                if (d.in <= 0 || d.out <= 0) return;
                std::vector<float> th((size_t)(d.in + 1) * d.ld);
                std::vector<unsigned char> w((size_t)(d.in + 1) * d.ldw * h->es), wt((size_t)d.out * d.ldt * h->es);
                HIP_OK(hipMemcpy(th.data(), (h->averaged ? h->ema_avg() : h->at<float>(h->off_theta)) + d.master, th.size() * 4, hipMemcpyDeviceToHost));
                HIP_OK(hipMemcpy(w.data(), h->at<void>(d.W), w.size(), hipMemcpyDeviceToHost));
                HIP_OK(hipMemcpy(wt.data(), h->at<void>(d.Wt), wt.size(), hipMemcpyDeviceToHost));
                float a = 0.f, b2 = 0.f;
                for (int r = 0; r <= d.in; ++r)
                    for (int c = 0; c < d.out; ++c) {
                        const float want = round_ct(th[(size_t)r * d.ld + c]);
                        a = std::max(a, std::fabs(elem(w, (size_t)r * d.ldw + c) - want));
                        b2 = std::max(b2, std::fabs(elem(wt, (size_t)c * d.ldt + r) - want));
                    }
                if (a > ew || b2 > et) worst = cnt;
                ew = std::max(ew, a); et = std::max(et, b2);
                ++cnt;
            };
            for (const Mod& md : h->mods) {
                for (const Dense& d : md.enc) check(d);
                check(md.head);
                for (const Dense& d : md.dec) check(d);
                check(md.outl);
                if (md.conv) { for (const ConvStage& st : md.cenc) check(st.d); for (const ConvStage& st : md.cdec) check(st.d); }
            }
            host_dst[0] = ew; host_dst[1] = et; host_dst[2] = (float)cnt; host_dst[3] = (float)worst;
            if (n_floats) *n_floats = 4;
            return;
        }
        else if (n == "ema_master") {
            if (!h->ema_on) throw Err("debug_fetch: parameter averaging is off");
            src = h->ema_avg(); cnt = h->P_int;
        }
        else if (n.rfind("mulv", 0) == 0 || n.rfind("g0_", 0) == 0) {
            const bool g0 = n[0] == 'g';
            const int m = std::atoi(n.c_str() + (g0 ? 3 : 4));
            if (m < 0 || m >= h->M) throw Err("debug_fetch: modality out of range");
            src = h->at<void>(g0 ? h->mods[m].g0 : h->mods[m].mulv); cnt = g0 ? (size_t)h->B * 3 * h->ld_eps : (size_t)h->B * 2 * h->nz;
        } else throw Err("debug_fetch: unknown tensor " + n);
        if (cnt > max_floats) throw Err("debug_fetch: destination too small");
        HIP_OK(hipDeviceSynchronize());
        HIP_OK(hipMemcpy(host_dst, src, cnt * 4, hipMemcpyDeviceToHost));
        if (n_floats) *n_floats = cnt;
    });
}

}
```

### vae_assoc_amd/csrc/avae_kernels.hip

```cpp
#include "avae_device.h"
#include "avae_complete.h"
#include <hip/hip_ext.h>
#include <stdexcept>
#include "../../include/avae.h"

namespace avae {

typedef __attribute__((ext_vector_type(8))) __bf16 bf16x8;
typedef __attribute__((ext_vector_type(4))) __bf16 bf16x4;
typedef __attribute__((ext_vector_type(4))) float f32x4;
typedef __attribute__((ext_vector_type(4))) unsigned u32x4;


template <typename CT> __device__ __forceinline__ CT to_ct(float v);
template <> __device__ __forceinline__ float to_ct<float>(float v) { return v; }
template <> __device__ __forceinline__ __bf16 to_ct<__bf16>(float v) { return (__bf16)v; }

__device__ __forceinline__ float bf16_bits_to_float(unsigned b) { return __uint_as_float(b << 16); }

template <typename CT> __device__ __forceinline__ void load4(const CT* p, float v[4]);
template <> __device__ __forceinline__ void load4<float>(const float* p, float v[4]) {
    float4 t = *reinterpret_cast<const float4*>(p);
    v[0] = t.x; v[1] = t.y; v[2] = t.z; v[3] = t.w;
}
// ... 1306 lines not shown
        const int nt = w.tiles_m * w.tiles_n;
        const int q = nt >> 3, r = nt & 7;
        if (idx >= q + (part < r ? 1 : 0)) return;
        t = (part < r ? part * (q + 1) : r * (q + 1) + (part - r) * q) + idx;
    }
    if (w.kind == K_LATENT) {
        latent_item<4, MASK>(w, t, red);
        AVAE_STAMP(4)
        AVAE_STAMP_FLUSH()
        return;
    }
    const int tid = threadIdx.x, lane = tid & 63, wave = __builtin_amdgcn_readfirstlane(tid >> 6);
    const int wr = wave >> 1, wc = wave & 1, fr = lane & 15, fq = lane >> 4;
    const int tm = t / w.tiles_n, tn = t - tm * w.tiles_n;
    const int m0 = tm * BM, n0 = tn * 32;
    const int nk = (w.K * ES) / kTileBytesK;
    typedef const __attribute__((address_space(1))) void* gp_t;
    typedef __attribute__((address_space(3))) void* lp_t;
    const int prow = wave * 8 + (lane >> 3), lc = ((lane & 7) ^ ((prow >> 1) & 7)) * 16;
    const unsigned char* srcA = reinterpret_cast<const unsigned char*>(w.A) + (size_t)(m0 + prow) * w.lda * ES + lc;
    const unsigned char* srcB = reinterpret_cast<const unsigned char*>(w.B) + (size_t)(n0 + prow) * w.ldb * ES + lc;
    const int orow = m0 + wr * 16 + fr, ocol = n0 + wc * 16 + 4 * fq;
    const f32x4 xq = *reinterpret_cast<const f32x4*>(reinterpret_cast<const float*>(w.aux0) + (size_t)min(orow, w.M - 1) * w.ldx + min(ocol, w.ldx - 4));
    const bool rpres = !MASK || w.present[(size_t)min(orow, w.M - 1) * w.present_ld] != 0;
#define AVAE_S_DMA(kt, buf)                                                                                             \
    { __builtin_amdgcn_global_load_lds((gp_t)(srcA + (size_t)(kt) * kTileBytesK), (lp_t)(smem + (buf) * kStage + wave * 1024), 16, 0, 0);          \
      __builtin_amdgcn_global_load_lds((gp_t)(srcB + (size_t)(kt) * kTileBytesK), (lp_t)(smem + (buf) * kStage + (4 + wave) * 1024), 16, 0, 0); }
    AVAE_STAMP(1)
    const int npro = nk < RING - 1 ? nk : RING - 1;
    for (int p = 0; p < npro; ++p) AVAE_S_DMA(p, p)
    const int sw0 = (fq ^ (fr >> 1)) * 16;
    const int aoff = (wr * 16 + fr) * kTileBytesK, boff = (32 + wc * 16 + fr) * kTileBytesK;
    f32x4 acc = {0.f, 0.f, 0.f, 0.f};
    int buf = 0;
    for (int kt = 0; kt < nk; ++kt) {
        const int rem = nk - 1 - kt;
        if (rem >= 2) asm volatile("s_waitcnt vmcnt(4)" ::: "memory");
        else if (rem == 1) asm volatile("s_waitcnt vmcnt(2)" ::: "memory");
        else asm volatile("s_waitcnt vmcnt(0)" ::: "memory");
        asm volatile("s_barrier" ::: "memory");
        if (kt == 0) { AVAE_STAMP(2) }
        const unsigned char* Sb = smem + buf * kStage;
        const u32x4 a0 = *reinterpret_cast<const u32x4*>(Sb + aoff + sw0), b0 = *reinterpret_cast<const u32x4*>(Sb + boff + sw0);
        const int fill = buf == 0 ? RING - 1 : buf - 1;
        if (kt + RING - 1 < nk) AVAE_S_DMA(kt + RING - 1, fill)
        const u32x4 a1 = *reinterpret_cast<const u32x4*>(Sb + aoff + (sw0 ^ 64)), b1 = *reinterpret_cast<const u32x4*>(Sb + boff + (sw0 ^ 64));
        mma<CT>(b0, a0, acc);
        mma<CT>(b1, a1, acc);
        buf = buf + 1 == RING ? 0 : buf + 1;
    }
#undef AVAE_S_DMA
    AVAE_STAMP(3)
    const float sc = w.scale;
    float csum = 0.0f, v[4];
#pragma unroll
    for (int e = 0; e < 4; ++e) {
        const bool ok = orow < w.M && ocol + e < w.N && rpres;
        float sl, da;
        if (w.binary) loss_bernoulli(acc[e], xq[e], sc, sl, da);
        else loss_gauss(acc[e], xq[e], sc, sl, da);
        csum += ok ? sl : 0.0f;
        v[e] = ok ? da : 0.0f;
    }
    if (orow < w.M && ocol < w.N) store_row<CT>(reinterpret_cast<CT*>(w.out0) + (size_t)orow * w.ld0 + ocol, v, w.N - ocol);
    const float total = block_sum<4>(csum, red);
    if (tid == 0) w.partial[w.slot_base + t] = total;
    AVAE_STAMP(4)
    AVAE_STAMP_FLUSH()
}
void launch_small_loss(int compute_dtype, const LaunchArgs& args, int grid_x, int grid_y, int lds_bytes, hipStream_t s, unsigned long long* stamps, int launch_id) {
    const dim3 grid(grid_x, grid_y), block(kThreads);
    bool masked = false;
    for (int i = 0; i < args.n_items; ++i) masked = masked || args.items[i].present != nullptr;
    if (masked) {
        if (compute_dtype == AVAE_BF16) AVAE_LAUNCH((k_small_loss<__bf16, true>), grid, block, lds_bytes, s, args, stamps, launch_id);
        else AVAE_LAUNCH((k_small_loss<float, true>), grid, block, lds_bytes, s, args, stamps, launch_id);
    } else if (compute_dtype == AVAE_BF16) AVAE_LAUNCH((k_small_loss<__bf16, false>), grid, block, lds_bytes, s, args, stamps, launch_id);
    else AVAE_LAUNCH((k_small_loss<float, false>), grid, block, lds_bytes, s, args, stamps, launch_id);
}

constexpr int kHeadStage = (32 + 64) * kTileBytesK, kHeadImg = 2 * 32 * kTileBytesK;
int small_head_lds_bytes() { return 4 * kHeadStage + kHeadImg + 64; }

template <typename CT> __device__ __forceinline__ void img_put(unsigned char* img, int row, int d, float v) {
    const int b = d * (int)sizeof(CT), bo = b & 127;
    *reinterpret_cast<CT*>(img + (b >> 7) * (32 * kTileBytesK) + row * kTileBytesK + ((((bo >> 4) ^ ((row >> 1) & 7)) << 4) | (bo & 15))) = to_ct<CT>(v);
}

template <typename CT, int ACT>
__global__ void __launch_bounds__(kThreads) k_small_latb(const LaunchArgs args, DevState* st, unsigned long long* stamps, int launch_id) {
    constexpr int RING = 4, ES = (int)sizeof(CT), TSL = ES == 2 ? 2 : 4;
    unsigned char* smem = avae_dyn_smem;
    unsigned char* img = smem + RING * kHeadStage;
    float* red = reinterpret_cast<float*>(img + kHeadImg);
#ifdef AVAE_STAMPS
    unsigned long long sv[kStampWords] = {0, 0, 0, 0, 0, 0, 0, 0};
#endif
    AVAE_STAMP(0)
    const int part = blockIdx.x & 7, idx = blockIdx.x >> 3;
    const WorkItem w = args.items[blockIdx.y];
    asm volatile("" :: "s"(w.A), "s"(w.B), "s"(w.out0), "s"(w.aux2), "s"(w.lda), "s"(w.ldb), "s"(w.K), "s"(w.ld0), "s"(w.tail_w), "s"(w.tail_out), "s"(w.tail_aux));
    int t;
    {
        const int nt = w.tiles_m * w.tiles_n;
        const int q = nt >> 3, r = nt & 7;
        if (idx >= q + (part < r ? 1 : 0)) return;
        t = (part < r ? part * (q + 1) : r * (q + 1) + (part - r) * q) + idx;
    }
    if (w.kind == K_COST) {
        cost_item<4>(w, st, red);
        AVAE_STAMP(4)
        AVAE_STAMP_FLUSH()
        return;
    }
    const int tid = threadIdx.x, lane = tid & 63, wave = __builtin_amdgcn_readfirstlane(tid >> 6);
    const int wr = wave >> 1, wc = wave & 1, fr = lane & 15, fq = lane >> 4;
    const int tm = t / w.tiles_n, ts = t - tm * w.tiles_n;
    const int m0 = tm * 32;
    const int nk = (w.K * ES) / kTileBytesK, nz = w.nz;
    typedef const __attribute__((address_space(1))) void* gp_t;
    typedef __attribute__((address_space(3))) void* lp_t;
    reinterpret_cast<f32x4*>(img)[tid] = f32x4{0.f, 0.f, 0.f, 0.f};
    reinterpret_cast<f32x4*>(img)[tid + kThreads] = f32x4{0.f, 0.f, 0.f, 0.f};
    const int orow = m0 + wr * 16 + fr;
    const int lde = (nz + 3) & ~3;
    const int t_i = wave & 1, t_c0 = (2 * ts + (wave >> 1)) * 32, t_sl = 2 * w.tail_kt;
    const int prow = wave * 8 + (lane >> 3), lc = ((lane & 7) ^ ((prow >> 1) & 7)) * 16;
    const unsigned char* srcA = reinterpret_cast<const unsigned char*>(w.A) + (size_t)(m0 + prow) * w.lda * ES + lc;
    const unsigned char* srcB = reinterpret_cast<const unsigned char*>(w.B) + (size_t)prow * w.ldb * ES + lc;
    const size_t b32 = (size_t)32 * w.ldb * ES;
#define AVAE_H_DMA(kt, buf)                                                                                             \
    { __builtin_amdgcn_global_load_lds((gp_t)(srcA + (size_t)(kt) * kTileBytesK), (lp_t)(smem + (buf) * kHeadStage + wave * 1024), 16, 0, 0);       \
      __builtin_amdgcn_global_load_lds((gp_t)(srcB + (size_t)(kt) * kTileBytesK), (lp_t)(smem + (buf) * kHeadStage + (4 + wave) * 1024), 16, 0, 0); \
      __builtin_amdgcn_global_load_lds((gp_t)(srcB + b32 + (size_t)(kt) * kTileBytesK), (lp_t)(smem + (buf) * kHeadStage + (8 + wave) * 1024), 16, 0, 0); }
    AVAE_STAMP(1)
    const int npro = nk < RING - 1 ? nk : RING - 1;
    for (int p = 0; p < npro; ++p) AVAE_H_DMA(p, p)
    constexpr int kExtra = 6 + 2 * TSL + 2;
    asm volatile("" ::: "memory"); __builtin_amdgcn_sched_barrier(0);
    f32x4 gm[2], gl[2], gf[2];
#pragma unroll
    for (int j = 0; j < 2; ++j) {
        const float* gr = reinterpret_cast<const float*>(w.aux2) + (size_t)min(orow, w.M - 1) * 3 * lde + min(wc * 32 + j * 16 + 4 * fq, lde - 4);
        gm[j] = *reinterpret_cast<const f32x4*>(gr); gl[j] = *reinterpret_cast<const f32x4*>(gr + lde); gf[j] = *reinterpret_cast<const f32x4*>(gr + 2 * lde);
    }
    u32x4 tb[TSL][2];
    typename Quad<CT>::raw ty[2];
#pragma unroll
    for (int j = 0; j < 2; ++j) {
        const unsigned char* pw = reinterpret_cast<const unsigned char*>(w.tail_w) + (size_t)min(t_c0 + 16 * j + fr, w.tail_n - 1) * w.tail_ldw * ES + fq * 16;
#pragma unroll
        for (int sl = 0; sl < TSL; ++sl) tb[sl][j] = *reinterpret_cast<const u32x4*>(pw + (sl < t_sl ? 64 * sl : 0));
        ty[j] = *reinterpret_cast<const typename Quad<CT>::raw*>(reinterpret_cast<const CT*>(w.tail_aux) + (size_t)min(m0 + 16 * t_i + fr, w.M - 1) * w.tail_ldx
                                                                   + min(t_c0 + 16 * j + 4 * fq, w.tail_ldx - 4));
    }
    asm volatile("" ::: "memory"); __builtin_amdgcn_sched_barrier(0);
    const int sw0 = (fq ^ (fr >> 1)) * 16;
    const int aoff = (wr * 16 + fr) * kTileBytesK, boff = (32 + wc * 32 + fr) * kTileBytesK;
    f32x4 acc[2] = {{0.f, 0.f, 0.f, 0.f}, {0.f, 0.f, 0.f, 0.f}};
    int buf = 0;
    for (int kt = 0; kt < nk; ++kt) {
        const int rem = nk - 1 - kt;
        if (kt < npro) {
            if (rem >= 2) asm volatile("s_waitcnt vmcnt(%0)" :: "n"(6 + kExtra) : "memory");
            else if (rem == 1) asm volatile("s_waitcnt vmcnt(%0)" :: "n"(3 + kExtra) : "memory");
            else asm volatile("s_waitcnt vmcnt(%0)" :: "n"(kExtra) : "memory");
        } else {
            if (rem >= 2) asm volatile("s_waitcnt vmcnt(6)" ::: "memory");
            else if (rem == 1) asm volatile("s_waitcnt vmcnt(3)" ::: "memory");
// ... 94 lines not shown
    const unsigned char* srcA = reinterpret_cast<const unsigned char*>(w.A) + (size_t)(m0 + prow) * w.lda * ES + lc;
    const unsigned char* srcB = reinterpret_cast<const unsigned char*>(w.B) + (size_t)prow * w.ldb * ES + lc;
    const size_t b32 = (size_t)32 * w.ldb * ES;
#define AVAE_H_DMA(kt, buf)                                                                                             \
    { __builtin_amdgcn_global_load_lds((gp_t)(srcA + (size_t)(kt) * kTileBytesK), (lp_t)(smem + (buf) * kHeadStage + wave * 1024), 16, 0, 0);       \
      __builtin_amdgcn_global_load_lds((gp_t)(srcB + (size_t)(kt) * kTileBytesK), (lp_t)(smem + (buf) * kHeadStage + (4 + wave) * 1024), 16, 0, 0); \
      __builtin_amdgcn_global_load_lds((gp_t)(srcB + b32 + (size_t)(kt) * kTileBytesK), (lp_t)(smem + (buf) * kHeadStage + (8 + wave) * 1024), 16, 0, 0); }
    AVAE_STAMP(1)
    const int npro = nk < RING - 1 ? nk : RING - 1;
    for (int p = 0; p < npro; ++p) AVAE_H_DMA(p, p)
    const int sw0 = (fq ^ (fr >> 1)) * 16;
    const int aoff = (wr * 16 + fr) * kTileBytesK, boff = (32 + wc * 32 + fr) * kTileBytesK;
    f32x4 acc[2] = {{0.f, 0.f, 0.f, 0.f}, {0.f, 0.f, 0.f, 0.f}};
    int buf = 0;
    for (int kt = 0; kt < nk; ++kt) {
        const int rem = nk - 1 - kt;
        if (rem >= 2) asm volatile("s_waitcnt vmcnt(6)" ::: "memory");
        else if (rem == 1) asm volatile("s_waitcnt vmcnt(3)" ::: "memory");
        else asm volatile("s_waitcnt vmcnt(0)" ::: "memory");
        asm volatile("s_barrier" ::: "memory");
        if (kt == 0) { AVAE_STAMP(2) }
        const unsigned char* Sb = smem + buf * kHeadStage;
        const u32x4 a0 = *reinterpret_cast<const u32x4*>(Sb + aoff + sw0);
        const u32x4 b00 = *reinterpret_cast<const u32x4*>(Sb + boff + sw0), b01 = *reinterpret_cast<const u32x4*>(Sb + boff + 16 * kTileBytesK + sw0);
        const int fill = buf == 0 ? RING - 1 : buf - 1;
        if (kt + RING - 1 < nk) AVAE_H_DMA(kt + RING - 1, fill)
        const u32x4 a1 = *reinterpret_cast<const u32x4*>(Sb + aoff + (sw0 ^ 64));
        const u32x4 b10 = *reinterpret_cast<const u32x4*>(Sb + boff + (sw0 ^ 64)), b11 = *reinterpret_cast<const u32x4*>(Sb + boff + 16 * kTileBytesK + (sw0 ^ 64));
        mma<CT>(b00, a0, acc[0]); mma<CT>(b01, a0, acc[1]);
        mma<CT>(b10, a1, acc[0]); mma<CT>(b11, a1, acc[1]);
        buf = buf + 1 == RING ? 0 : buf + 1;
    }
#undef AVAE_H_DMA
    lds_barrier();
    AVAE_STAMP(3)
    {
        const int orow = m0 + wr * 16 + fr, lrow = wr * 16 + fr;
        float* mulv = reinterpret_cast<float*>(w.out0) + (size_t)orow * w.ld0;
        const bool store = ts == 0 && orow < w.M;
#pragma unroll
        for (int j = 0; j < 2; ++j) {
            const int c0 = wc * 32 + j * 16 + 4 * fq;
            *reinterpret_cast<f32x4*>(MV + lrow * LDM + c0) = acc[j];
            if (store) {
#pragma unroll
                for (int e = 0; e < 4; ++e) if (c0 + e < 2 * nz) mulv[c0 + e] = acc[j][e];
            }
        }
    }
    lds_barrier();
    AVAE_STAMP(5)
    {
        CT* Z = reinterpret_cast<CT*>(w.out1) + (size_t)(m0 + zrow) * w.ld1;
        const bool store = ts == 0 && m0 + zrow < w.M;
#pragma unroll
        for (int e = 0; e < 4; ++e) {
            const int d = 4 * zg + e;
            if (d < nz) {
                const float z = __builtin_fmaf(fexp(0.5f * MV[zrow * LDM + nz + d]), ev[e], MV[zrow * LDM + d]);
                img_put<CT>(img, zrow, d, z);
                if (store) Z[d] = to_ct<CT>(z);
            }
        }
        if (tid < 32) img_put<CT>(img, tid, nz, 1.0f);
    }
    lds_barrier();
    AVAE_STAMP_EP(6)
    {
        const int arow = 16 * t_i + fr;
        f32x4 tacc[1][2] = {{{0.f, 0.f, 0.f, 0.f}, {0.f, 0.f, 0.f, 0.f}}};
#pragma unroll
        for (int sl = 0; sl < TSL; ++sl)
            if (TSL == 2 || sl < t_sl) {
                const u32x4 ta = *reinterpret_cast<const u32x4*>(img + (sl >> 1) * (32 * kTileBytesK) + arow * kTileBytesK + (((fq + 4 * (sl & 1)) ^ ((arow >> 1) & 7)) << 4));
                mma<CT>(tb[sl][0], ta, tacc[0][0]);
                mma<CT>(tb[sl][1], ta, tacc[0][1]);
            }
        regep_store<CT, 1, 2>(tacc, reinterpret_cast<CT*>(w.tail_out), w.tail_ldo, w.M, w.tail_n, m0 + arow, t_c0, lane,
            [&](int, int, int, float v) { return act_fwd_t<ACT>(v); });
    }
    AVAE_STAMP(4)
    AVAE_STAMP_FLUSH()
}
void launch_small_head(int compute_dtype, int act, const LaunchArgs& args, int grid_x, int grid_y, int lds_bytes, hipStream_t s,
                       unsigned long long* stamps, int launch_id) {
    const dim3 grid(grid_x, grid_y), block(kThreads);
#define K_HEAD_B(A) k_small_head<__bf16, A>
#define K_HEAD_F(A) k_small_head<float, A>
    if (compute_dtype == AVAE_BF16) {
        switch (act) {
            case AVAE_ACT_RELU: AVAE_LAUNCH((K_HEAD_B(AVAE_ACT_RELU)), grid, block, lds_bytes, s, args, stamps, launch_id); break;
            case AVAE_ACT_SOFTPLUS: AVAE_LAUNCH((K_HEAD_B(AVAE_ACT_SOFTPLUS)), grid, block, lds_bytes, s, args, stamps, launch_id); break;
            case AVAE_ACT_SIGMOID: AVAE_LAUNCH((K_HEAD_B(AVAE_ACT_SIGMOID)), grid, block, lds_bytes, s, args, stamps, launch_id); break;
            case AVAE_ACT_TANH: AVAE_LAUNCH((K_HEAD_B(AVAE_ACT_TANH)), grid, block, lds_bytes, s, args, stamps, launch_id); break;
            default: AVAE_LAUNCH((K_HEAD_B(AVAE_ACT_IDENTITY)), grid, block, lds_bytes, s, args, stamps, launch_id); break;
        }
    } else {
        switch (act) {
            case AVAE_ACT_RELU: AVAE_LAUNCH((K_HEAD_F(AVAE_ACT_RELU)), grid, block, lds_bytes, s, args, stamps, launch_id); break;
            case AVAE_ACT_SOFTPLUS: AVAE_LAUNCH((K_HEAD_F(AVAE_ACT_SOFTPLUS)), grid, block, lds_bytes, s, args, stamps, launch_id); break;
            case AVAE_ACT_SIGMOID: AVAE_LAUNCH((K_HEAD_F(AVAE_ACT_SIGMOID)), grid, block, lds_bytes, s, args, stamps, launch_id); break;
            case AVAE_ACT_TANH: AVAE_LAUNCH((K_HEAD_F(AVAE_ACT_TANH)), grid, block, lds_bytes, s, args, stamps, launch_id); break;
            default: AVAE_LAUNCH((K_HEAD_F(AVAE_ACT_IDENTITY)), grid, block, lds_bytes, s, args, stamps, launch_id); break;
        }
    }
#undef K_HEAD_B
#undef K_HEAD_F
}
void launch_small_latb(int compute_dtype, int act, const LaunchArgs& args, int grid_x, int grid_y, int lds_bytes, DevState* st, hipStream_t s,
                       unsigned long long* stamps, int launch_id) {
    const dim3 grid(grid_x, grid_y), block(kThreads);
#define K_LATB_B(A) k_small_latb<__bf16, A>
#define K_LATB_F(A) k_small_latb<float, A>
    if (compute_dtype == AVAE_BF16) {
        switch (act) {
            case AVAE_ACT_RELU: AVAE_LAUNCH((K_LATB_B(AVAE_ACT_RELU)), grid, block, lds_bytes, s, args, st, stamps, launch_id); break;
            case AVAE_ACT_SOFTPLUS: AVAE_LAUNCH((K_LATB_B(AVAE_ACT_SOFTPLUS)), grid, block, lds_bytes, s, args, st, stamps, launch_id); break;
            case AVAE_ACT_SIGMOID: AVAE_LAUNCH((K_LATB_B(AVAE_ACT_SIGMOID)), grid, block, lds_bytes, s, args, st, stamps, launch_id); break;
            case AVAE_ACT_TANH: AVAE_LAUNCH((K_LATB_B(AVAE_ACT_TANH)), grid, block, lds_bytes, s, args, st, stamps, launch_id); break;
            default: AVAE_LAUNCH((K_LATB_B(AVAE_ACT_IDENTITY)), grid, block, lds_bytes, s, args, st, stamps, launch_id); break;
        }
    } else {
        switch (act) {
            case AVAE_ACT_RELU: AVAE_LAUNCH((K_LATB_F(AVAE_ACT_RELU)), grid, block, lds_bytes, s, args, st, stamps, launch_id); break;
            case AVAE_ACT_SOFTPLUS: AVAE_LAUNCH((K_LATB_F(AVAE_ACT_SOFTPLUS)), grid, block, lds_bytes, s, args, st, stamps, launch_id); break;
            case AVAE_ACT_SIGMOID: AVAE_LAUNCH((K_LATB_F(AVAE_ACT_SIGMOID)), grid, block, lds_bytes, s, args, st, stamps, launch_id); break;
            case AVAE_ACT_TANH: AVAE_LAUNCH((K_LATB_F(AVAE_ACT_TANH)), grid, block, lds_bytes, s, args, st, stamps, launch_id); break;
            default: AVAE_LAUNCH((K_LATB_F(AVAE_ACT_IDENTITY)), grid, block, lds_bytes, s, args, st, stamps, launch_id); break;
        }
    }
#undef K_LATB_B
#undef K_LATB_F
}

template <typename CT, bool ADAM>
__global__ void __launch_bounds__(kThreads) k_small_tn(const TnLaunchArgs args, unsigned long long* stamps, int launch_id) {
    constexpr int BM = 64, RING = 4, ES = (int)sizeof(CT), EPR = kTileBytesK / ES, NCH = 4;
    constexpr int kStage = 2 * BM * kTileBytesK;
    unsigned char* smem = avae_dyn_smem;
#ifdef AVAE_STAMPS
    unsigned long long sv[kStampWords] = {0, 0, 0, 0, 0, 0, 0, 0};
#endif
    AVAE_STAMP(0)
    const int part = blockIdx.x & 7, idx = blockIdx.x >> 3;
    int entry = blockIdx.y, t_piece = -1;
    if (args.xcd_pieces) {
        const TnPiece* row = args.pieces[part];
        int e = 0, lo = 0;
#pragma unroll
        for (int i = 0; i < kTnPieces; ++i) { const int ce = row[i].cum_end; if (idx >= ce) { e = i + 1; lo = ce; } }
        if (e >= kTnPieces) return;
        entry = row[e].item; t_piece = row[e].tile_off + idx - lo;
    }
    const TnItem w = args.items[entry];
    asm volatile("" :: "s"(w.A), "s"(w.B), "s"(w.out), "s"(w.lda), "s"(w.ldb), "s"(w.K), "s"(w.ld0), "s"(w.tile_off));
    float lr_t = 0.f;
    if constexpr (ADAM) lr_t = args.st->lr_t;
    int t;
    if (t_piece >= 0) {
        t = t_piece;
    } else {
        const int nt = w.tile_cnt;
        const int q = nt >> 3, r = nt & 7;
        if (idx >= q + (part < r ? 1 : 0)) return;
        t = (part < r ? part * (q + 1) : r * (q + 1) + (part - r) * q) + idx + w.tile_off;
    }
    const int tid = threadIdx.x, lane = tid & 63, wave = __builtin_amdgcn_readfirstlane(tid >> 6);
    const int wr = wave >> 1, wc = wave & 1, fr = lane & 15, fq = lane >> 4;
    const int tm = t / w.tiles_n, tn = t - tm * w.tiles_n;
    const int m0 = tm * BM, n0 = tn * BM;
    const int nk = (w.K * ES) / kTileBytesK;
    typedef const __attribute__((address_space(1))) void* gp_t;
    typedef __attribute__((address_space(3))) void* lp_t;
    const unsigned char* src[NCH];
    size_t kadv[NCH];
#pragma unroll
    for (int c = 0; c < NCH; ++c) {
        const int r = (c * 4 + wave) * 8 + (lane >> 3);
        const bool is_a = c < 2;
        const int rr = is_a ? r : r - BM, sub = rr / EPR, k = rr - sub * EPR;
        const int lc = (lane & 7) ^ tn_swz<CT>(k);
        const size_t ld_b = (size_t)(is_a ? w.lda : w.ldb) * ES;
        kadv[c] = (size_t)EPR * ld_b;
        src[c] = reinterpret_cast<const unsigned char*>(is_a ? w.A : w.B) + (size_t)(is_a ? m0 : n0) * ES + (size_t)k * ld_b + (size_t)sub * kTileBytesK + lc * 16;
    }
#define AVAE_T_DMA(kt, buf)                                                                                             \
    { _Pragma("unroll") for (int c = 0; c < NCH; ++c)                                                                   \
        __builtin_amdgcn_global_load_lds((gp_t)(src[c] + (size_t)(kt) * kadv[c]), (lp_t)(smem + (buf) * kStage + (c * 4 + wave) * 1024), 16, 0, 0); }
    int offA[2], offB[2];
#pragma unroll
    for (int i = 0; i < 2; ++i) { offA[i] = tn_frag_off<CT>(wr * 32 + i * 16, lane); offB[i] = BM * kTileBytesK + tn_frag_off<CT>(wc * 32 + i * 16, lane); }
    AVAE_STAMP(1)
    const int npro = nk < RING - 1 ? nk : RING - 1;
    for (int p = 0; p < npro; ++p) AVAE_T_DMA(p, p)
    const int c4 = (tid & 15) * 4;
    f32x4 pth[4], pmm[4], pvv[4];
    auto fetch_state = [&]() {
#pragma unroll
        for (int k = 0; k < 4; ++k) {
            const int grow = m0 + (tid >> 4) + 16 * k, gcol = n0 + c4;
            const bool ok = grow < w.M && gcol < w.N;
            const float* gp = w.out + (size_t)(ok ? grow : m0) * w.ld0 + (ok ? gcol : n0);
            pth[k] = *reinterpret_cast<const f32x4*>(gp + args.d_theta);
            pmm[k] = *reinterpret_cast<const f32x4*>(gp + args.d_m);
            pvv[k] = *reinterpret_cast<const f32x4*>(gp + args.d_v);
        }
    };
    f32x4 acc[2][2];
#pragma unroll
    for (int i = 0; i < 2; ++i)
#pragma unroll
        for (int j = 0; j < 2; ++j) acc[i][j] = f32x4{0.f, 0.f, 0.f, 0.f};
    int buf = 0;
    for (int kt = 0; kt < nk; ++kt) {
        const int rem = nk - 1 - kt;
        if (rem >= 2) asm volatile("s_waitcnt vmcnt(8)" ::: "memory");
        else if (rem == 1) asm volatile("s_waitcnt vmcnt(4)" ::: "memory");
        else asm volatile("s_waitcnt vmcnt(0)" ::: "memory");
        asm volatile("s_barrier" ::: "memory");
        if (kt == 0) { AVAE_STAMP(2) }
        const unsigned char* Sb = smem + buf * kStage;
        u32x4 a0[2], b0[2], a1[2], b1[2];
#pragma unroll
        for (int i = 0; i < 2; ++i) { a0[i] = tn_frag<CT>(Sb, offA[i], 0); b0[i] = tn_frag<CT>(Sb, offB[i], 0); }
        const int fill = buf == 0 ? RING - 1 : buf - 1;
        if (kt + RING - 1 < nk) AVAE_T_DMA(kt + RING - 1, fill)
#pragma unroll
        for (int i = 0; i < 2; ++i) { a1[i] = tn_frag<CT>(Sb, offA[i], 1); b1[i] = tn_frag<CT>(Sb, offB[i], 1); }
        if constexpr (sizeof(CT) == 2) { tn_wait_lds(); tn_frags_ready(a0); tn_frags_ready(b0); tn_frags_ready(a1); tn_frags_ready(b1); }
#pragma unroll
        for (int i = 0; i < 2; ++i)
#pragma unroll
            for (int j = 0; j < 2; ++j) mma<CT>(b0[j], a0[i], acc[i][j]);
#pragma unroll
        for (int i = 0; i < 2; ++i)
#pragma unroll
            for (int j = 0; j < 2; ++j) mma<CT>(b1[j], a1[i], acc[i][j]);
        buf = buf + 1 == RING ? 0 : buf + 1;
    }
#undef AVAE_T_DMA
    AVAE_STAMP(3)
    if constexpr (!ADAM) {
#pragma unroll
        for (int i = 0; i < 2; ++i) {
            const int row = m0 + wr * 32 + i * 16 + fr;
#pragma unroll
            for (int j = 0; j < 2; ++j) {
                const int col = n0 + wc * 32 + j * 16 + 4 * fq;
                if (row < w.M && col < w.N) {
                    const float g[4] = {acc[i][j][0], acc[i][j][1], acc[i][j][2], acc[i][j][3]};
                    store_row<float>(w.out + (size_t)row * w.ld0 + col, g, w.N - col);
                }
            }
        }
    } else {
        constexpr int LDT = 65;
        float* T = reinterpret_cast<float*>(smem);
        fetch_state();
        lds_barrier();
#pragma unroll
        for (int i = 0; i < 2; ++i)
#pragma unroll
            for (int j = 0; j < 2; ++j)
#pragma unroll
                for (int e = 0; e < 4; ++e) T[(wr * 32 + i * 16 + fr) * LDT + wc * 32 + j * 16 + 4 * fq + e] = acc[i][j][e];
        lds_barrier();
        const float omb1 = 1.0f - args.beta1, omb2 = 1.0f - args.beta2;
        const int r4 = (tid & 15) * 4;
        float g[4][4], th[4][4], m[4][4], v[4][4];
#pragma unroll
        for (int k = 0; k < 4; ++k) {
            const int r = (tid >> 4) + 16 * k;
#pragma unroll
            for (int e = 0; e < 4; ++e) { g[k][e] = T[r * LDT + c4 + e]; th[k][e] = pth[k][e]; m[k][e] = pmm[k][e]; v[k][e] = pvv[k][e]; }
#pragma unroll
            for (int e = 0; e < 4; ++e) adam_update(g[k][e], m[k][e], v[k][e], th[k][e], omb1, omb2, lr_t, args.eps);
#pragma unroll
            for (int e = 0; e < 4; ++e) T[r * LDT + c4 + e] = th[k][e];
        }
        const bool full = m0 + BM <= w.M && n0 + BM <= w.N;
        auto store_group = [&](int k, float* gp, CT* wp) {
            store4<float>(gp, g[k]);
            store4<float>(gp + args.d_theta, th[k]); store4<float>(gp + args.d_m, m[k]); store4<float>(gp + args.d_v, v[k]);
            store4<CT>(wp, th[k]);
        };
        if (full) {
#pragma unroll
            for (int k = 0; k < 4; ++k) {
                const int grow = m0 + (tid >> 4) + 16 * k, gcol = n0 + c4;
                store_group(k, w.out + (size_t)grow * w.ld0 + gcol, reinterpret_cast<CT*>(w.W) + (size_t)grow * w.ldw + gcol);
            }
        } else {
#pragma unroll
            for (int k = 0; k < 4; ++k) {
                const int grow = m0 + (tid >> 4) + 16 * k, gcol = n0 + c4;
                float* gp = w.out + (size_t)grow * w.ld0 + gcol;
                CT* wp = reinterpret_cast<CT*>(w.W) + (size_t)grow * w.ldw + gcol;
                const int nv = w.N - gcol;
                if (grow < w.M && nv >= 4) {
                    store_group(k, gp, wp);
                } else if (grow < w.M && nv > 0) {
#pragma unroll
                    for (int e = 0; e < 3; ++e) if (e < nv) {
                        gp[e] = g[k][e]; gp[args.d_theta + e] = th[k][e]; gp[args.d_m + e] = m[k][e]; gp[args.d_v + e] = v[k][e]; wp[e] = to_ct<CT>(th[k][e]);
                    }
                    asm volatile("; partial quad" ::: "memory");
                }
            }
        }
        lds_barrier();
#pragma unroll
        for (int k = 0; k < 4; ++k) {
            const int c = (tid >> 4) + 16 * k;
            const int gcol = n0 + c, grow = m0 + r4;
            float t[4];
#pragma unroll
            for (int e = 0; e < 4; ++e) t[e] = T[(r4 + e) * LDT + c];
            CT* tp = reinterpret_cast<CT*>(w.Wt) + (size_t)gcol * w.ldt + grow;
            if (full) store4<CT>(tp, t);
            else if (gcol < w.N && grow < w.M) store_row<CT>(tp, t, w.M - grow);
        }
    }
    AVAE_STAMP(4)
    AVAE_STAMP_FLUSH()
}
void launch_small_tn(int compute_dtype, const TnLaunchArgs& args, int grid_x, int grid_y, hipStream_t s, unsigned long long* stamps, int launch_id) {
    const dim3 grid(grid_x, grid_y), block(kThreads);
    const int lds_bytes = 4 * 2 * 64 * kTileBytesK;
    if (compute_dtype == AVAE_BF16) {
        if (args.adam) AVAE_LAUNCH((k_small_tn<__bf16, true>), grid, block, lds_bytes, s, args, stamps, launch_id);
        else AVAE_LAUNCH((k_small_tn<__bf16, false>), grid, block, lds_bytes, s, args, stamps, launch_id);
    } else {
        if (args.adam) AVAE_LAUNCH((k_small_tn<float, true>), grid, block, lds_bytes, s, args, stamps, launch_id);
        else AVAE_LAUNCH((k_small_tn<float, false>), grid, block, lds_bytes, s, args, stamps, launch_id);
    }
}

template <typename CT, int KIND>
static void launch_small_act(int act, const LaunchArgs& args, dim3 grid, int lds_bytes, hipStream_t s, unsigned long long* stamps, int launch_id) {
    const dim3 block(kThreads);
    switch (act) {
        case AVAE_ACT_RELU: AVAE_LAUNCH((k_small<CT, KIND, AVAE_ACT_RELU>), grid, block, lds_bytes, s, args, stamps, launch_id); break;
        case AVAE_ACT_SOFTPLUS: AVAE_LAUNCH((k_small<CT, KIND, AVAE_ACT_SOFTPLUS>), grid, block, lds_bytes, s, args, stamps, launch_id); break;
        case AVAE_ACT_SIGMOID: AVAE_LAUNCH((k_small<CT, KIND, AVAE_ACT_SIGMOID>), grid, block, lds_bytes, s, args, stamps, launch_id); break;
        case AVAE_ACT_TANH: AVAE_LAUNCH((k_small<CT, KIND, AVAE_ACT_TANH>), grid, block, lds_bytes, s, args, stamps, launch_id); break;
        default: AVAE_LAUNCH((k_small<CT, KIND, AVAE_ACT_IDENTITY>), grid, block, lds_bytes, s, args, stamps, launch_id); break;
    }
}
void launch_small(int compute_dtype, const LaunchArgs& args, int grid_x, int grid_y, int lds_bytes, hipStream_t s, unsigned long long* stamps, int launch_id) {
    const dim3 grid(grid_x, grid_y);
    const int kind = args.items[0].kind == K_DGRAD_HIDDEN ? 1 : 0, act = args.items[0].act;
    if (args.items[0].kind == K_FWD_OUT_STORE) {
        const dim3 block(kThreads);
        if (compute_dtype == AVAE_BF16) AVAE_LAUNCH((k_small<__bf16, 2, AVAE_ACT_IDENTITY>), grid, block, lds_bytes, s, args, stamps, launch_id);
        else AVAE_LAUNCH((k_small<float, 2, AVAE_ACT_IDENTITY>), grid, block, lds_bytes, s, args, stamps, launch_id);
        return;
    }
    if (compute_dtype == AVAE_BF16) { if (kind) launch_small_act<__bf16, 1>(act, args, grid, lds_bytes, s, stamps, launch_id); else launch_small_act<__bf16, 0>(act, args, grid, lds_bytes, s, stamps, launch_id); }
    else { if (kind) launch_small_act<float, 1>(act, args, grid, lds_bytes, s, stamps, launch_id); else launch_small_act<float, 0>(act, args, grid, lds_bytes, s, stamps, launch_id); }
}

template <typename CT, int ACT>
__global__ void __launch_bounds__(kThreads) k_chain2(const LaunchArgs args, unsigned* counters, unsigned* err) {
    constexpr int BM = 32, RING = 4, ES = (int)sizeof(CT);
    constexpr int kStage = 64 * kTileBytesK;
    unsigned char* smem = avae_dyn_smem;
    const int part = blockIdx.x & 7, idx = blockIdx.x >> 3, half = args.n_items >> 1;
    const WorkItem w1 = args.items[blockIdx.y], w2 = args.items[half + blockIdx.y];
    asm volatile("" :: "s"(w1.A), "s"(w1.B), "s"(w1.out0), "s"(w1.lda), "s"(w1.ldb), "s"(w1.K), "s"(w1.ld0), "s"(w2.B), "s"(w2.out0), "s"(w2.ldb), "s"(w2.K), "s"(w2.ld0));
    int t;
    {
        const int nt = w1.tiles_m * w1.tiles_n;
        const int q = nt >> 3, r = nt & 7;
        if (idx >= q + (part < r ? 1 : 0)) return;
        t = (part < r ? part * (q + 1) : r * (q + 1) + (part - r) * q) + idx;
    }
    const int tid = threadIdx.x, lane = tid & 63, wave = __builtin_amdgcn_readfirstlane(tid >> 6);
    const int wr = wave >> 1, wc = wave & 1, fr = lane & 15, fq = lane >> 4;
    const int tm = t / w1.tiles_n, tn = t - tm * w1.tiles_n;
    const int m0 = tm * BM, n0 = tn * 32;
    typedef const __attribute__((address_space(1))) void* gp_t;
    typedef __attribute__((address_space(3))) void* lp_t;
    const int prow = wave * 8 + (lane >> 3), lc = ((lane & 7) ^ ((prow >> 1) & 7)) * 16;
    const int sw0 = (fq ^ (fr >> 1)) * 16;
    const int aoff = (wr * 16 + fr) * kTileBytesK, boff = (32 + wc * 16 + fr) * kTileBytesK;
    const int orow = m0 + wr * 16 + fr, ocol = n0 + wc * 16 + 4 * fq;
    f32x4 acc;
#define AVAE_C_LOOP(W, AUX)                                                                                               \
    {                                                                                                                     \
        const unsigned char* srcA = reinterpret_cast<const unsigned char*>((W).A) + (size_t)(m0 + prow) * (W).lda * ES + lc;   \
        const unsigned char* srcB = reinterpret_cast<const unsigned char*>((W).B) + (size_t)(n0 + prow) * (W).ldb * ES + lc;   \
        const int nk = ((W).K * ES) / kTileBytesK;                                                                        \
        auto dma = [&](int kt, int buf) __attribute__((always_inline)) {                                                  \
            __builtin_amdgcn_global_load_lds((gp_t)(srcA + (size_t)kt * kTileBytesK), (lp_t)(smem + buf * kStage + wave * 1024), 16, 0, AUX);       \
            __builtin_amdgcn_global_load_lds((gp_t)(srcB + (size_t)kt * kTileBytesK), (lp_t)(smem + buf * kStage + (4 + wave) * 1024), 16, 0, 0); };  \
        const int npro = nk < RING - 1 ? nk : RING - 1;                                                                   \
        for (int p = 0; p < npro; ++p) dma(p, p);                                                                         \
        acc = f32x4{0.f, 0.f, 0.f, 0.f};                                                                                  \
        int buf = 0;                                                                                                      \
        for (int kt = 0; kt < nk; ++kt) {                                                                                 \
            const int rem = nk - 1 - kt;                                                                                  \
            if (rem >= 2) asm volatile("s_waitcnt vmcnt(4)" ::: "memory");                                                \
            else if (rem == 1) asm volatile("s_waitcnt vmcnt(2)" ::: "memory");                                           \
            else asm volatile("s_waitcnt vmcnt(0)" ::: "memory");                                                         \
            asm volatile("s_barrier" ::: "memory");                                                                       \
            const unsigned char* Sb = smem + buf * kStage;                                                                 \
            const u32x4 a0 = *reinterpret_cast<const u32x4*>(Sb + aoff + sw0), b0 = *reinterpret_cast<const u32x4*>(Sb + boff + sw0);   \
            const int fill = buf == 0 ? RING - 1 : buf - 1;                                                               \
            if (kt + RING - 1 < nk) dma(kt + RING - 1, fill);                                                             \
            const u32x4 a1 = *reinterpret_cast<const u32x4*>(Sb + aoff + (sw0 ^ 64)), b1 = *reinterpret_cast<const u32x4*>(Sb + boff + (sw0 ^ 64)); \
            mma<CT>(b0, a0, acc);                                                                                         \
            mma<CT>(b1, a1, acc);                                                                                         \
            buf = buf + 1 == RING ? 0 : buf + 1;                                                                          \
        }                                                                                                                 \
    }
    AVAE_C_LOOP(w1, 0)
// ... 1771 lines not shown
```

Baseline: 4.743 million.

## Compact TN descriptors, 16-row head kernels, and skip grad stores in fused wgrad-Adam

Adds a compact packed descriptor form for the fused wgrad+Adam TN kernel, so each block resolves its piece from a few scalar loads of kernel arguments instead of indexing the full item table. Adds 16-row variants of the small head and latent kernels for narrow heads, which launch more, smaller blocks. Drops the fp32 gradient store in the fused Adam epilogue on every multi-step graph iteration except the last. The skipped store means intermediate gradients are not available in memory, and the extra code paths add complexity.

```diff
diff --git a/vae_assoc_amd/csrc/avae_device.h b/vae_assoc_amd/csrc/avae_device.h
--- a/vae_assoc_amd/csrc/avae_device.h
+++ b/vae_assoc_amd/csrc/avae_device.h
@@ -126,6 +126,24 @@
 constexpr int kMaxTnItems = 32;
 constexpr int kTnPieces = 8;
 struct TnPiece { unsigned short item, tile_off, cum_end, pad; };
+struct TnDesc {
+    unsigned long long q[4];
+};
+struct TnTail {
+    float* out; void* W; void* Wt;
+    int M, N, ld0, ldw, ldt, pad;
+};
+constexpr int kTnLayers = 24;
+__host__ __device__ inline TnDesc tn_desc(const void* A, const void* B, unsigned lda, unsigned ldb, unsigned tiles_n, unsigned tile_off,
+                                          unsigned cum_end, unsigned layer) {
+    TnDesc d;
+    d.q[0] = (unsigned long long)(size_t)A; d.q[1] = (unsigned long long)(size_t)B;
+    d.q[2] = (unsigned long long)lda | (unsigned long long)ldb << 32;
+    d.q[3] = (unsigned long long)(tiles_n & 0xffffu) | (unsigned long long)(tile_off & 0xffffu) << 16 | (unsigned long long)(cum_end & 0xffffu) << 32
+             | (unsigned long long)(layer & 0xffffu) << 48;
+    return d;
+}
+__host__ __device__ inline int tn_desc_cum_end(const TnDesc& d) { return (int)((d.q[3] >> 32) & 0xffffu); }
 struct DevState;
 struct TnLaunchArgs {
     int n_items;
@@ -138,10 +156,16 @@
     const DevState* st;
     const ConvA* conv_tab;
     int xcd_pieces;
-    TnPiece pieces[8][kTnPieces];
-    TnItem items[kMaxTnItems];
+    int tn_k;
+    union {
+        struct { TnPiece pieces[8][kTnPieces]; TnItem items[kMaxTnItems]; };
+        struct { TnDesc desc[8][kTnPieces]; TnTail tails[kTnLayers]; };
+    };
 };
 static_assert(sizeof(TnLaunchArgs) <= 4096, "kernel arguments are passed by value: 4 KiB");
+static_assert(sizeof(TnDesc) == 32 && sizeof(TnTail) == 48, "one XCD's descriptors are four 64-byte scalar loads");
+static_assert(sizeof(TnDesc) * 8 * kTnPieces + sizeof(TnTail) * kTnLayers <= sizeof(TnPiece) * 8 * kTnPieces + sizeof(TnItem) * kMaxTnItems,
+              "the compact form fits the bytes of pieces[] + items[]");
 
 struct DevState {
     long long step;
@@ -463,9 +487,10 @@
 void launch_fill(void* base, int elem_bytes, unsigned bits, long long start, long long stride, int count, hipStream_t s);
 void launch_sums(const ReduceArgs& a, int n_blocks, hipStream_t s);
 int small_head_lds_bytes();
-void launch_small_latb(int compute_dtype, int act, const LaunchArgs& args, int grid_x, int grid_y, int lds_bytes, DevState* st, hipStream_t s,
+int small_head16_lds_bytes();
+void launch_small_latb(int compute_dtype, int act, int rows, const LaunchArgs& args, int grid_x, int grid_y, int lds_bytes, DevState* st, hipStream_t s,
                        unsigned long long* stamps, int launch_id);
-void launch_small_head(int compute_dtype, int act, const LaunchArgs& args, int grid_x, int grid_y, int lds_bytes, hipStream_t s,
+void launch_small_head(int compute_dtype, int act, int rows, const LaunchArgs& args, int grid_x, int grid_y, int lds_bytes, hipStream_t s,
                        unsigned long long* stamps, int launch_id);
 void launch_small_tn(int compute_dtype, const TnLaunchArgs& args, int grid_x, int grid_y, hipStream_t s, unsigned long long* stamps, int launch_id);
 void launch_small_loss(int compute_dtype, const LaunchArgs& args, int grid_x, int grid_y, int lds_bytes, hipStream_t s, unsigned long long* stamps, int launch_id);
diff --git a/vae_assoc_amd/csrc/avae_host.hip b/vae_assoc_amd/csrc/avae_host.hip
--- a/vae_assoc_amd/csrc/avae_host.hip
+++ b/vae_assoc_amd/csrc/avae_host.hip
@@ -216,6 +216,7 @@
     std::vector<Launch> bwd;
     std::vector<Launch> wgrad;
     std::vector<Launch> wgrad_adam;
+    std::vector<Launch> wgrad_adam_lean;
     int n_buckets = 1;
     int bwd_split = 0;
     std::vector<Launch> wgrad_b[2];
@@ -288,6 +289,10 @@
     unsigned draw_id = 0;
     bool timing = false;
     bool debug_sync = false;
+    bool no_tn_compact = false;
+    bool head_rows32 = false;
+    long wgrad_routes[2] = {0, 0};
+    bool keep_grad_stores = false;
     std::vector<std::string> tnames;
     std::vector<TimingRec> trecs;
 
@@ -1092,7 +1097,7 @@
 
 void dp_ranges(const avae_handle* h, int* n_buckets, std::vector<avae_handle::Range> (&out)[2]);
 
-void xcd_pieces(Launch& L) {
+void xcd_pieces(Launch& L, bool compact) {
     TnLaunchArgs& a = L.targs;
     std::vector<TnItem> layers;
     for (int i = 0; i < a.n_items; ++i) {
@@ -1134,15 +1139,38 @@
         }
     }
     int longest = 0;
-    for (int b = 0; b < 8; ++b) {
-        longest = std::max(longest, bins[b].load);
-        for (int i = 0; i < kTnPieces; ++i)
-            a.pieces[b][i] = i < (int)bins[b].pc.size() ? bins[b].pc[i] : TnPiece{0, 0, (unsigned short)bins[b].load, 0};
-    }
-    std::memset(a.items, 0, sizeof(a.items));
-    for (size_t i = 0; i < layers.size(); ++i) a.items[i] = layers[i];
+    for (int b = 0; b < 8; ++b) longest = std::max(longest, bins[b].load);
+    compact = compact && a.adam && (int)layers.size() <= kTnLayers && quota <= 65535;
+    for (const TnItem& l : layers)
+        compact = compact && l.K == layers[0].K && l.tiles_n <= 65535 && l.lda >= 0 && l.ldb >= 0 && l.conv == 0 && l.ksplit <= 1 && l.bias_row == 0;
+    if (compact) {
+        std::memset(a.desc, 0, sizeof(a.desc));
+        std::memset(a.tails, 0, sizeof(a.tails));
+        for (int b = 0; b < 8; ++b)
+            for (int i = 0; i < kTnPieces; ++i) {
+                if (i < (int)bins[b].pc.size()) {
+                    const TnPiece& pc = bins[b].pc[i];
+                    const TnItem& l = layers[pc.item];
+                    a.desc[b][i] = tn_desc(l.A, l.B, (unsigned)l.lda, (unsigned)l.ldb, (unsigned)l.tiles_n, pc.tile_off, pc.cum_end, pc.item);
+                } else {
+                    a.desc[b][i] = tn_desc(nullptr, nullptr, 0, 0, 0, 0, (unsigned)bins[b].load, 0);
+                }
+            }
+        for (size_t i = 0; i < layers.size(); ++i) {
+            const TnItem& l = layers[i];
+            a.tails[i] = TnTail{l.out, l.W, l.Wt, l.M, l.N, l.ld0, l.ldw, l.ldt, 0};
+        }
+        a.tn_k = layers[0].K;
+        a.xcd_pieces = 2;
+    } else {
+        for (int b = 0; b < 8; ++b)
+            for (int i = 0; i < kTnPieces; ++i)
+                a.pieces[b][i] = i < (int)bins[b].pc.size() ? bins[b].pc[i] : TnPiece{0, 0, (unsigned short)bins[b].load, 0};
+        std::memset(a.items, 0, sizeof(a.items));
+        for (size_t i = 0; i < layers.size(); ++i) a.items[i] = layers[i];
+        a.xcd_pieces = 1;
+    }
     a.n_items = (int)layers.size();
-    a.xcd_pieces = 1;
     L.grid_x = 8 * longest; L.grid_y = 1; L.blocks = L.grid_x;
     a.grid_x = L.grid_x;
 }
@@ -1210,6 +1238,27 @@
             if (lean && mode == 1)
                 for (int k = 0; k < Lp.count; ++k) lean = lean && h->items[Lp.first + k].kind == K_FWD_HEAD && h->items[Lp.first + k].out1 != nullptr;
             if (lean) { Lp.cfg = mode == 2 ? 10 : 11; Lp.lds = small_head_lds_bytes(); Lp.lean_act = act; }
+            if (lean && !h->head_rows32) {
+                long tiles = 0;
+                bool fits = true;
+                for (int k = 0; k < Lp.count; ++k) {
+                    const WorkItem& n = h->items[Lp.first + k];
+                    if (n.kind == K_COST) continue;
+                    fits = fits && 2 * n.nz <= 48;
+                    tiles += (long)n.tiles_m * n.tiles_n;
+                }
+                if (fits && tiles <= 128) {
+                    int mt = 1;
+                    for (int k = 0; k < Lp.count; ++k) {
+                        for (WorkItem* n : {&h->items[Lp.first + k], &Lp.args.items[k]}) {
+                            if (n->kind != K_COST) n->tiles_m = (n->M + 15) / 16;
+                            mt = std::max(mt, n->tiles_m * n->tiles_n);
+                        }
+                    }
+                    Lp.cfg = mode == 2 ? 14 : 15; Lp.lds = small_head16_lds_bytes();
+                    Lp.grid_x = (mt + 7) & ~7; Lp.blocks = Lp.grid_x * Lp.grid_y; Lp.args.grid_x = Lp.grid_x;
+                }
+            }
         }
         return true;
     };
@@ -1683,7 +1732,7 @@
             if (base > 0) h->wgrad.push_back(L);
         }
     }
-    h->wgrad_adam.clear();
+    h->wgrad_adam.clear(); h->wgrad_adam_lean.clear();
     if (!any_conv && h->wgrad.size() == 1 && h->wgrad[0].tn && h->wgrad[0].cfg == 0 && h->wgrad[0].targs.xcd_group == 1
         && !std::getenv("AVAE_NO_LEAN") && !std::getenv("AVAE_NO_ADAM_FUSE")) {
         Launch L = h->wgrad[0];
@@ -1710,8 +1759,10 @@
             L.targs.d_v = h->at<float>(h->off_v) - h->grad();
             L.targs.beta1 = h->cfg.beta1; L.targs.beta2 = h->cfg.beta2; L.targs.eps = h->cfg.adam_eps;
             L.targs.st = h->state();
-            if (!std::getenv("AVAE_NO_XCD_PIECES")) xcd_pieces(L);
+            if (!std::getenv("AVAE_NO_XCD_PIECES")) xcd_pieces(L, !h->no_tn_compact);
             h->wgrad_adam.push_back(L);
+            L.targs.adam = 2;
+            h->wgrad_adam_lean.push_back(L);
         }
     }
     if (!std::getenv("AVAE_NO_WARM")) {
@@ -1899,7 +1950,16 @@
         if (w.present) w.present += (size_t)j * h->pres_set;
         if (hyper && (w.kind == K_LATENT || (w.kind == K_COST && w.bump_step))) w.tail_w = hyper + j;
     }
-    for (int i = 0; i < L.targs.n_items && L.type == 0; ++i) { TnItem& t = L.targs.items[i]; fix(t.A); fix(t.B); fix(t.out); }
+    if (L.targs.xcd_pieces == 2) {
+        for (int b = 0; b < 8 && L.type == 0; ++b)
+            for (int i = 0; i < kTnPieces; ++i)
+                for (int k = 0; k < 2; ++k) {
+                    const unsigned char* q = reinterpret_cast<const unsigned char*>((size_t)L.targs.desc[b][i].q[k]);
+                    fix(q);
+                    L.targs.desc[b][i].q[k] = (unsigned long long)(size_t)q;
+                }
+    } else
+        for (int i = 0; i < L.targs.n_items && L.type == 0; ++i) { TnItem& t = L.targs.items[i]; fix(t.A); fix(t.B); fix(t.out); }
     for (int i = 0; i < L.ga.n_seg && L.type == 1; ++i) fix(L.ga.seg[i].src);
     return L;
 }
@@ -1916,8 +1976,8 @@
     else if (L.type == 8) launch_rowsum(h->cfg.compute_dtype, L.rs, L.blocks, s);
     else if (L.type == 9) launch_sums(L.ra, L.blocks, s);
     else if (L.cfg == 13) launch_chain2(h->cfg.compute_dtype, L.args, L.grid_x, L.grid_y, L.lds, h->at<unsigned>(h->off_chain), h->at<unsigned>(h->off_chain) + kMaxMod * 64, s);
-    else if (L.cfg == 11) launch_small_head(h->cfg.compute_dtype, L.lean_act, L.args, L.grid_x, L.grid_y, L.lds, s, stamps, stamp);
-    else if (L.cfg == 10) launch_small_latb(h->cfg.compute_dtype, L.lean_act, L.args, L.grid_x, L.grid_y, L.lds, h->state(), s, stamps, stamp);
+    else if (L.cfg == 11 || L.cfg == 15) launch_small_head(h->cfg.compute_dtype, L.lean_act, L.cfg == 15 ? 16 : 32, L.args, L.grid_x, L.grid_y, L.lds, s, stamps, stamp);
+    else if (L.cfg == 10 || L.cfg == 14) launch_small_latb(h->cfg.compute_dtype, L.lean_act, L.cfg == 14 ? 16 : 32, L.args, L.grid_x, L.grid_y, L.lds, h->state(), s, stamps, stamp);
     else if (L.cfg == 9) launch_small_loss(h->cfg.compute_dtype, L.args, L.grid_x, L.grid_y, L.lds, s, stamps, stamp);
     else if (L.cfg == 7) launch_small(h->cfg.compute_dtype, L.args, L.grid_x, L.grid_y, L.lds, s, stamps, stamp);
     else if (L.tn && L.cfg == 12) launch_small_tn(h->cfg.compute_dtype, L.targs, L.grid_x, L.grid_y, s, stamps, stamp);
@@ -1926,6 +1986,8 @@
     LAUNCH_OK(L.name);
     if (h->debug_sync) {
         std::fprintf(stderr, "[avae] launch %s type=%d cfg=%d items=%d blocks=%d\n", L.name.c_str(), L.type, L.cfg, L.count, L.blocks);
+        if (L.tn && L.cfg == 12)
+            std::fprintf(stderr, "        tn lookup=%s layers=%d\n", L.targs.xcd_pieces == 2 ? "compact" : L.targs.xcd_pieces == 1 ? "pieces" : "grid", L.targs.n_items);
         for (int i = 0; i < L.args.n_items && L.type == 0; ++i)
             std::fprintf(stderr, "        item kind=%d M=%d N=%d K=%d lda=%d ldb=%d tiles=%dx%d\n", L.args.items[i].kind, L.args.items[i].M,
                          L.args.items[i].N, L.args.items[i].K, L.args.items[i].lda, L.args.items[i].ldb, L.args.items[i].tiles_m, L.args.items[i].tiles_n);
@@ -2128,12 +2190,15 @@
     LAUNCH_OK("fill");
 }
 
-void step_body(avae_handle* h, const std::vector<Launch>& fwd, hipStream_t s, int j, int stamp_base = -1) {
+void step_body(avae_handle* h, const std::vector<Launch>& fwd, hipStream_t s, int j, int stamp_base = -1, bool store_g = true) {
     auto sb = [&](size_t k) { return stamp_base < 0 ? -1 : stamp_base + (int)k; };
     run_set(h, fwd, 0, fwd.size(), j, s, stamp_base, true);
     run_set(h, h->bwd, 0, h->bwd.size(), j, s, sb(fwd.size()), true);
     if (!h->wgrad_adam.empty() && !h->clip_on && !h->ema_on) {
-        run_set(h, h->wgrad_adam, 0, h->wgrad_adam.size(), j, s, sb(fwd.size() + h->bwd.size()), true);
+        const bool lean = !store_g && !h->keep_grad_stores;
+        const std::vector<Launch>& ls = lean ? h->wgrad_adam_lean : h->wgrad_adam;
+        ++h->wgrad_routes[lean ? 1 : 0];
+        run_set(h, ls, 0, ls.size(), j, s, sb(fwd.size() + h->bwd.size()), true);
         return;
     }
     run_set(h, h->wgrad, 0, h->wgrad.size(), j, s, sb(fwd.size() + h->bwd.size()), true);
@@ -2150,7 +2215,7 @@
         }, true);
         for (int gi = 0; gi < 2; ++gi) p.multi[gi] = capture(h, [&](hipStream_t cs) {
             run_prep_batch(h, x0.data(), nullptr, nullptr, h->B, kTrainSalt, cs, present, kMultiSizes[gi]);
-            for (int j = 0; j < kMultiSizes[gi]; ++j) step_body(h, p.fwd, cs, j);
+            for (int j = 0; j < kMultiSizes[gi]; ++j) step_body(h, p.fwd, cs, j, -1, j == kMultiSizes[gi] - 1);
         }, true);
     } catch (...) { p.full.release(); p.multi[0].release(); p.multi[1].release(); throw; }
 }
@@ -3051,6 +3116,9 @@
         h->cfg = *cfg;
         if (const char* e = std::getenv("AVAE_DEBUG_SYNC")) h->debug_sync = e[0] == '1';
         if (h->debug_sync) h->cfg.use_graph = 0;
+        if (const char* e = std::getenv("AVAE_KEEP_GRAD_STORES")) h->keep_grad_stores = e[0] == '1';
+        if (const char* e = std::getenv("AVAE_NO_TN_COMPACT")) h->no_tn_compact = e[0] == '1';
+        if (const char* e = std::getenv("AVAE_HEAD_ROWS")) h->head_rows32 = std::atoi(e) == 32;
         if (h->cfg.beta1 == 0.f && h->cfg.beta2 == 0.f && h->cfg.adam_eps == 0.f) { h->cfg.beta1 = 0.9f; h->cfg.beta2 = 0.999f; h->cfg.adam_eps = 1e-8f; }
         int ndev = 0;
         HIP_OK(hipGetDeviceCount(&ndev));
@@ -4077,21 +4145,7 @@
         std::string n(name ? name : "");
         const void* src = nullptr;
         size_t cnt = 0;
-        if (n == "eps") {
-            cnt = (size_t)h->B * h->nz;
-            if (cnt > max_floats) throw Err("debug_fetch: destination too small");
-            HIP_OK(hipDeviceSynchronize());
-            HIP_OK(hipMemcpy2D(host_dst, (size_t)h->nz * 4, h->at<void>(h->off_eps), (size_t)h->ld_eps * 4, (size_t)h->nz * 4, h->B, hipMemcpyDeviceToHost));
-            if (n_floats) *n_floats = cnt;
-            return;
-        }
-#ifdef AVAE_STAMPS
-        else if (n == "stamps") { src = h->at<void>(h->off_stamps); cnt = (size_t)kStampLaunches * kStampBlocks * kStampWords * 2; }
-#endif
-        else if ((n[0] == 'E' || n[0] == 'D') && n.size() >= 4 && n.find('_') != std::string::npos) {
-            const int m = std::atoi(n.c_str() + 1), k = std::atoi(n.c_str() + n.find('_') + 1);
-            if (m < 0 || m >= h->M || h->mods[m].conv || k < 0 || k >= h->mods[m].L) throw Err("debug_fetch: no such hidden layer");
-            const Act& a = n[0] == 'E' ? h->mods[m].E[k] : h->mods[m].D[k];
+        auto dense_act = [&](const Act& a) {
             cnt = (size_t)h->B * a.width;
             if (cnt > max_floats) throw Err("debug_fetch: destination too small");
             HIP_OK(hipDeviceSynchronize());
@@ -4105,6 +4159,28 @@
                     host_dst[(size_t)r * a.width + c] = v;
                 }
             if (n_floats) *n_floats = cnt;
+        };
+        if (n == "eps") {
+            cnt = (size_t)h->B * h->nz;
+            if (cnt > max_floats) throw Err("debug_fetch: destination too small");
+            HIP_OK(hipDeviceSynchronize());
+            HIP_OK(hipMemcpy2D(host_dst, (size_t)h->nz * 4, h->at<void>(h->off_eps), (size_t)h->ld_eps * 4, (size_t)h->nz * 4, h->B, hipMemcpyDeviceToHost));
+            if (n_floats) *n_floats = cnt;
+            return;
+        }
+#ifdef AVAE_STAMPS
+        else if (n == "stamps") { src = h->at<void>(h->off_stamps); cnt = (size_t)kStampLaunches * kStampBlocks * kStampWords * 2; }
+#endif
+        else if ((n[0] == 'E' || n[0] == 'D') && n.size() >= 4 && n.find('_') != std::string::npos) {
+            const int m = std::atoi(n.c_str() + 1), k = std::atoi(n.c_str() + n.find('_') + 1);
+            if (m < 0 || m >= h->M || h->mods[m].conv || k < 0 || k >= h->mods[m].L) throw Err("debug_fetch: no such hidden layer");
+            dense_act(n[0] == 'E' ? h->mods[m].E[k] : h->mods[m].D[k]);
+            return;
+        }
+        else if ((n[0] == 'Z' || n.rfind("dH", 0) == 0) && std::isdigit((unsigned char)n[n[0] == 'Z' ? 1 : 2])) {
+            const int m = std::atoi(n.c_str() + (n[0] == 'Z' ? 1 : 2));
+            if (m < 0 || m >= h->M) throw Err("debug_fetch: modality out of range");
+            dense_act(n[0] == 'Z' ? h->mods[m].Z : h->mods[m].dH);
             return;
         }
         else if ((n[0] == 'X' || n[0] == 'T') && n.size() >= 2 && std::isdigit((unsigned char)n[1])) {
@@ -4175,6 +4251,12 @@
             if (n_floats) *n_floats = 4;
             return;
         }
+        else if (n == "wgrad_routes") {
+            if (max_floats < 2) throw Err("debug_fetch: destination too small");
+            host_dst[0] = (float)h->wgrad_routes[0]; host_dst[1] = (float)h->wgrad_routes[1];
+            if (n_floats) *n_floats = 2;
+            return;
+        }
         else if (n == "ema_master") {
             if (!h->ema_on) throw Err("debug_fetch: parameter averaging is off");
             src = h->ema_avg(); cnt = h->P_int;
diff --git a/vae_assoc_amd/csrc/avae_kernels.hip b/vae_assoc_amd/csrc/avae_kernels.hip
--- a/vae_assoc_amd/csrc/avae_kernels.hip
+++ b/vae_assoc_amd/csrc/avae_kernels.hip
@@ -1412,9 +1412,9 @@
 constexpr int kHeadStage = (32 + 64) * kTileBytesK, kHeadImg = 2 * 32 * kTileBytesK;
 int small_head_lds_bytes() { return 4 * kHeadStage + kHeadImg + 64; }
 
-template <typename CT> __device__ __forceinline__ void img_put(unsigned char* img, int row, int d, float v) {
+template <typename CT, int ROWS = 32> __device__ __forceinline__ void img_put(unsigned char* img, int row, int d, float v) {
     const int b = d * (int)sizeof(CT), bo = b & 127;
-    *reinterpret_cast<CT*>(img + (b >> 7) * (32 * kTileBytesK) + row * kTileBytesK + ((((bo >> 4) ^ ((row >> 1) & 7)) << 4) | (bo & 15))) = to_ct<CT>(v);
+    *reinterpret_cast<CT*>(img + (b >> 7) * (ROWS * kTileBytesK) + row * kTileBytesK + ((((bo >> 4) ^ ((row >> 1) & 7)) << 4) | (bo & 15))) = to_ct<CT>(v);
 }
 
 template <typename CT, int ACT>
@@ -1675,11 +1675,263 @@
     AVAE_STAMP(4)
     AVAE_STAMP_FLUSH()
 }
-void launch_small_head(int compute_dtype, int act, const LaunchArgs& args, int grid_x, int grid_y, int lds_bytes, hipStream_t s,
+constexpr int kHead16Stage = (16 + 48) * kTileBytesK, kHead16Img = 2 * 16 * kTileBytesK;
+int small_head16_lds_bytes() { return 4 * kHead16Stage + kHead16Img + 64; }
+
+template <typename CT, int ACT>
+__global__ void __launch_bounds__(kThreads) k_small_latb16(const LaunchArgs args, DevState* st, unsigned long long* stamps, int launch_id) {
+    constexpr int RING = 4, ES = (int)sizeof(CT), TSL = ES == 2 ? 2 : 4;
+    unsigned char* smem = avae_dyn_smem;
+    unsigned char* img = smem + RING * kHead16Stage;
+    float* red = reinterpret_cast<float*>(img + kHead16Img);
+#ifdef AVAE_STAMPS
+    unsigned long long sv[kStampWords] = {0, 0, 0, 0, 0, 0, 0, 0};
+#endif
+    AVAE_STAMP(0)
+    const int part = blockIdx.x & 7, idx = blockIdx.x >> 3;
+    const WorkItem w = args.items[blockIdx.y];
+    asm volatile("" :: "s"(w.A), "s"(w.B), "s"(w.out0), "s"(w.aux2), "s"(w.lda), "s"(w.ldb), "s"(w.K), "s"(w.ld0), "s"(w.tail_w), "s"(w.tail_out), "s"(w.tail_aux));
+    int t;
+    {
+        const int nt = w.tiles_m * w.tiles_n;
+        const int q = nt >> 3, r = nt & 7;
+        if (idx >= q + (part < r ? 1 : 0)) return;
+        t = (part < r ? part * (q + 1) : r * (q + 1) + (part - r) * q) + idx;
+    }
+    if (w.kind == K_COST) {
+        cost_item<4>(w, st, red);
+        AVAE_STAMP(4)
+        AVAE_STAMP_FLUSH()
+        return;
+    }
+    const int tid = threadIdx.x, lane = tid & 63, wave = __builtin_amdgcn_readfirstlane(tid >> 6);
+    const int cb = wave < 3 ? wave : 2, fr = lane & 15, fq = lane >> 4;
+    const int tm = t / w.tiles_n, ts = t - tm * w.tiles_n;
+    const int m0 = tm * 16;
+    const int nk = (w.K * ES) / kTileBytesK, nz = w.nz;
+    typedef const __attribute__((address_space(1))) void* gp_t;
+    typedef __attribute__((address_space(3))) void* lp_t;
+    reinterpret_cast<f32x4*>(img)[tid] = f32x4{0.f, 0.f, 0.f, 0.f};
+    const int orow = m0 + fr;
+    const int lde = (nz + 3) & ~3;
+    const int t_c0 = (2 * ts + (wave & 1)) * 32, t_sl = 2 * w.tail_kt;
+    const int prow = wave * 8 + (lane >> 3), lc = ((lane & 7) ^ ((prow >> 1) & 7)) * 16;
+    const unsigned char* src0 = wave < 2 ? reinterpret_cast<const unsigned char*>(w.A) + (size_t)(m0 + prow) * w.lda * ES + lc
+                                         : reinterpret_cast<const unsigned char*>(w.B) + (size_t)(prow - 16) * w.ldb * ES + lc;
+    const unsigned char* src1 = reinterpret_cast<const unsigned char*>(w.B) + (size_t)(prow + 16) * w.ldb * ES + lc;
+#define AVAE_H_DMA(kt, buf)                                                                                             \
+    { __builtin_amdgcn_global_load_lds((gp_t)(src0 + (size_t)(kt) * kTileBytesK), (lp_t)(smem + (buf) * kHead16Stage + wave * 1024), 16, 0, 0);       \
+      __builtin_amdgcn_global_load_lds((gp_t)(src1 + (size_t)(kt) * kTileBytesK), (lp_t)(smem + (buf) * kHead16Stage + (4 + wave) * 1024), 16, 0, 0); }
+    AVAE_STAMP(1)
+    const int npro = nk < RING - 1 ? nk : RING - 1;
+    for (int p = 0; p < npro; ++p) AVAE_H_DMA(p, p)
+    constexpr int kExtra = 3 + 2 * TSL + 2;
+    asm volatile("" ::: "memory"); __builtin_amdgcn_sched_barrier(0);
+    f32x4 gm, gl, gf;
+    {
+        const float* gr = reinterpret_cast<const float*>(w.aux2) + (size_t)min(orow, w.M - 1) * 3 * lde + min(cb * 16 + 4 * fq, lde - 4);
+        gm = *reinterpret_cast<const f32x4*>(gr); gl = *reinterpret_cast<const f32x4*>(gr + lde); gf = *reinterpret_cast<const f32x4*>(gr + 2 * lde);
+    }
+    u32x4 tb[TSL][2];
+    typename Quad<CT>::raw ty[2];
+#pragma unroll
+    for (int j = 0; j < 2; ++j) {
+        const unsigned char* pw = reinterpret_cast<const unsigned char*>(w.tail_w) + (size_t)min(t_c0 + 16 * j + fr, w.tail_n - 1) * w.tail_ldw * ES + fq * 16;
+#pragma unroll
+        for (int sl = 0; sl < TSL; ++sl) tb[sl][j] = *reinterpret_cast<const u32x4*>(pw + (sl < t_sl ? 64 * sl : 0));
+        ty[j] = *reinterpret_cast<const typename Quad<CT>::raw*>(reinterpret_cast<const CT*>(w.tail_aux) + (size_t)min(m0 + fr, w.M - 1) * w.tail_ldx
+                                                                   + min(t_c0 + 16 * j + 4 * fq, w.tail_ldx - 4));
+    }
+    asm volatile("" ::: "memory"); __builtin_amdgcn_sched_barrier(0);
+    const int sw0 = (fq ^ (fr >> 1)) * 16;
+    const int aoff = fr * kTileBytesK, boff = (16 + cb * 16 + fr) * kTileBytesK;
+    f32x4 acc = {0.f, 0.f, 0.f, 0.f};
+    int buf = 0;
+    for (int kt = 0; kt < nk; ++kt) {
+        const int rem = nk - 1 - kt;
+        if (kt < npro) {
+            if (rem >= 2) asm volatile("s_waitcnt vmcnt(%0)" :: "n"(4 + kExtra) : "memory");
+            else if (rem == 1) asm volatile("s_waitcnt vmcnt(%0)" :: "n"(2 + kExtra) : "memory");
+            else asm volatile("s_waitcnt vmcnt(%0)" :: "n"(kExtra) : "memory");
+        } else {
+            if (rem >= 2) asm volatile("s_waitcnt vmcnt(4)" ::: "memory");
+            else if (rem == 1) asm volatile("s_waitcnt vmcnt(2)" ::: "memory");
+            else asm volatile("s_waitcnt vmcnt(0)" ::: "memory");
+        }
+        asm volatile("s_barrier" ::: "memory");
+        if (kt == 0) { AVAE_STAMP(2) }
+        const unsigned char* Sb = smem + buf * kHead16Stage;
+        u32x4 a0 = {0, 0, 0, 0}, b0 = {0, 0, 0, 0};
+        if (wave < 3) { a0 = *reinterpret_cast<const u32x4*>(Sb + aoff + sw0); b0 = *reinterpret_cast<const u32x4*>(Sb + boff + sw0); }
+        const int fill = buf == 0 ? RING - 1 : buf - 1;
+        if (kt + RING - 1 < nk) AVAE_H_DMA(kt + RING - 1, fill)
+        if (wave < 3) {
+            const u32x4 a1 = *reinterpret_cast<const u32x4*>(Sb + aoff + (sw0 ^ 64)), b1 = *reinterpret_cast<const u32x4*>(Sb + boff + (sw0 ^ 64));
+            mma<CT>(b0, a0, acc);
+            mma<CT>(b1, a1, acc);
+        }
+        buf = buf + 1 == RING ? 0 : buf + 1;
+    }
+#undef AVAE_H_DMA
+    asm volatile("" :: "v"(gm), "v"(gl), "v"(gf), "v"(ty[0]), "v"(ty[1]));
+#pragma unroll
+    for (int sl = 0; sl < TSL; ++sl) asm volatile("" :: "v"(tb[sl][0]), "v"(tb[sl][1]));
+    AVAE_STAMP(3)
+    if (wave < 3) {
+        CT* dH = reinterpret_cast<CT*>(w.out0) + (size_t)orow * w.ld0;
+        const bool store = ts == 0 && orow < w.M;
+#pragma unroll
+        for (int e = 0; e < 4; ++e) {
+            const int d = cb * 16 + 4 * fq + e;
+            if (d < nz) {
+                const float dz = acc[e];
+                const float dmu = dz + gm[e], dlv = __builtin_fmaf(dz, gf[e], gl[e]);
+                img_put<CT, 16>(img, fr, d, dmu);
+                img_put<CT, 16>(img, fr, nz + d, dlv);
+                if (store) { dH[d] = to_ct<CT>(dmu); dH[nz + d] = to_ct<CT>(dlv); }
+            }
+        }
+    }
+    lds_barrier();
+    AVAE_STAMP(5)
+    if (wave < 2) {
+        f32x4 tacc[1][2] = {{{0.f, 0.f, 0.f, 0.f}, {0.f, 0.f, 0.f, 0.f}}};
+#pragma unroll
+        for (int sl = 0; sl < TSL; ++sl)
+            if (TSL == 2 || sl < t_sl) {
+                const u32x4 ta = *reinterpret_cast<const u32x4*>(img + (sl >> 1) * (16 * kTileBytesK) + fr * kTileBytesK + (((fq + 4 * (sl & 1)) ^ ((fr >> 1) & 7)) << 4));
+                mma<CT>(tb[sl][0], ta, tacc[0][0]);
+                mma<CT>(tb[sl][1], ta, tacc[0][1]);
+            }
+        regep_store<CT, 1, 2>(tacc, reinterpret_cast<CT*>(w.tail_out), w.tail_ldo, w.M, w.tail_n, m0 + fr, t_c0, lane,
+            [&](int, int j, int r, float v) { return v * act_bwd_t<ACT>(quad_elem<CT>(ty[j], r)); });
+    }
+    AVAE_STAMP(4)
+    AVAE_STAMP_FLUSH()
+}
+template <typename CT, int ACT>
+__global__ void __launch_bounds__(kThreads) k_small_head16(const LaunchArgs args, unsigned long long* stamps, int launch_id) {
+    constexpr int RING = 4, ES = (int)sizeof(CT), TSL = ES == 2 ? 2 : 4, LDM = 52;
+    unsigned char* smem = avae_dyn_smem;
+    unsigned char* img = smem + RING * kHead16Stage;
+    float* MV = reinterpret_cast<float*>(smem);
+#ifdef AVAE_STAMPS
+    unsigned long long sv[kStampWords] = {0, 0, 0, 0, 0, 0, 0, 0};
+#endif
+    AVAE_STAMP(0)
+    const int part = blockIdx.x & 7, idx = blockIdx.x >> 3;
+    const WorkItem w = args.items[blockIdx.y];
+    asm volatile("" :: "s"(w.A), "s"(w.B), "s"(w.out0), "s"(w.out1), "s"(w.aux0), "s"(w.lda), "s"(w.ldb), "s"(w.K), "s"(w.ld0), "s"(w.tail_w), "s"(w.tail_out));
+    int t;
+    {
+        const int nt = w.tiles_m * w.tiles_n;
+        const int q = nt >> 3, r = nt & 7;
+        if (idx >= q + (part < r ? 1 : 0)) return;
+        t = (part < r ? part * (q + 1) : r * (q + 1) + (part - r) * q) + idx;
+    }
+    const int tid = threadIdx.x, lane = tid & 63, wave = __builtin_amdgcn_readfirstlane(tid >> 6);
+    const int cb = wave < 3 ? wave : 2, fr = lane & 15, fq = lane >> 4;
+    const int tm = t / w.tiles_n, ts = t - tm * w.tiles_n;
+    const int m0 = tm * 16;
+    const int nk = (w.K * ES) / kTileBytesK, nz = w.nz;
+    typedef const __attribute__((address_space(1))) void* gp_t;
+    typedef __attribute__((address_space(3))) void* lp_t;
+    reinterpret_cast<f32x4*>(img)[tid] = f32x4{0.f, 0.f, 0.f, 0.f};
+    const int zrow = tid >> 4, zg = tid & 15;
+    const f32x4 ev = *reinterpret_cast<const f32x4*>(reinterpret_cast<const float*>(w.aux0) + (size_t)min(m0 + zrow, w.M - 1) * w.ldx + min(4 * zg, w.ldx - 4));
+    const int t_c0 = (2 * ts + (wave & 1)) * 32, t_sl = 2 * w.tail_kt;
+    u32x4 tb[TSL][2];
+#pragma unroll
+    for (int j = 0; j < 2; ++j) {
+        const unsigned char* pw = reinterpret_cast<const unsigned char*>(w.tail_w) + (size_t)min(t_c0 + 16 * j + fr, w.tail_n - 1) * w.tail_ldw * ES + fq * 16;
+#pragma unroll
+        for (int sl = 0; sl < TSL; ++sl) if (TSL == 2 || sl < t_sl) tb[sl][j] = *reinterpret_cast<const u32x4*>(pw + 64 * sl);
+    }
+    const int prow = wave * 8 + (lane >> 3), lc = ((lane & 7) ^ ((prow >> 1) & 7)) * 16;
+    const unsigned char* src0 = wave < 2 ? reinterpret_cast<const unsigned char*>(w.A) + (size_t)(m0 + prow) * w.lda * ES + lc
+                                         : reinterpret_cast<const unsigned char*>(w.B) + (size_t)(prow - 16) * w.ldb * ES + lc;
+    const unsigned char* src1 = reinterpret_cast<const unsigned char*>(w.B) + (size_t)(prow + 16) * w.ldb * ES + lc;
+#define AVAE_H_DMA(kt, buf)                                                                                             \
+    { __builtin_amdgcn_global_load_lds((gp_t)(src0 + (size_t)(kt) * kTileBytesK), (lp_t)(smem + (buf) * kHead16Stage + wave * 1024), 16, 0, 0);       \
+      __builtin_amdgcn_global_load_lds((gp_t)(src1 + (size_t)(kt) * kTileBytesK), (lp_t)(smem + (buf) * kHead16Stage + (4 + wave) * 1024), 16, 0, 0); }
+    AVAE_STAMP(1)
+    const int npro = nk < RING - 1 ? nk : RING - 1;
+    for (int p = 0; p < npro; ++p) AVAE_H_DMA(p, p)
+    const int sw0 = (fq ^ (fr >> 1)) * 16;
+    const int aoff = fr * kTileBytesK, boff = (16 + cb * 16 + fr) * kTileBytesK;
+    f32x4 acc = {0.f, 0.f, 0.f, 0.f};
+    int buf = 0;
+    for (int kt = 0; kt < nk; ++kt) {
+        const int rem = nk - 1 - kt;
+        if (rem >= 2) asm volatile("s_waitcnt vmcnt(4)" ::: "memory");
+        else if (rem == 1) asm volatile("s_waitcnt vmcnt(2)" ::: "memory");
+        else asm volatile("s_waitcnt vmcnt(0)" ::: "memory");
+        asm volatile("s_barrier" ::: "memory");
+        if (kt == 0) { AVAE_STAMP(2) }
+        const unsigned char* Sb = smem + buf * kHead16Stage;
+        u32x4 a0 = {0, 0, 0, 0}, b0 = {0, 0, 0, 0};
+        if (wave < 3) { a0 = *reinterpret_cast<const u32x4*>(Sb + aoff + sw0); b0 = *reinterpret_cast<const u32x4*>(Sb + boff + sw0); }
+        const int fill = buf == 0 ? RING - 1 : buf - 1;
+        if (kt + RING - 1 < nk) AVAE_H_DMA(kt + RING - 1, fill)
+        if (wave < 3) {
+            const u32x4 a1 = *reinterpret_cast<const u32x4*>(Sb + aoff + (sw0 ^ 64)), b1 = *reinterpret_cast<const u32x4*>(Sb + boff + (sw0 ^ 64));
+            mma<CT>(b0, a0, acc);
+            mma<CT>(b1, a1, acc);
+        }
+        buf = buf + 1 == RING ? 0 : buf + 1;
+    }
+#undef AVAE_H_DMA
+    lds_barrier();
+    AVAE_STAMP(3)
+    if (wave < 3) {
+        const int orow = m0 + fr;
+        float* mulv = reinterpret_cast<float*>(w.out0) + (size_t)orow * w.ld0;
+        const bool store = ts == 0 && orow < w.M;
+        const int c0 = cb * 16 + 4 * fq;
+        *reinterpret_cast<f32x4*>(MV + fr * LDM + c0) = acc;
+        if (store) {
+#pragma unroll
+            for (int e = 0; e < 4; ++e) if (c0 + e < 2 * nz) mulv[c0 + e] = acc[e];
+        }
+    }
+    lds_barrier();
+    AVAE_STAMP(5)
+    {
+        CT* Z = reinterpret_cast<CT*>(w.out1) + (size_t)(m0 + zrow) * w.ld1;
+        const bool store = ts == 0 && m0 + zrow < w.M;
+#pragma unroll
+        for (int e = 0; e < 4; ++e) {
+            const int d = 4 * zg + e;
+            if (d < nz) {
+                const float z = __builtin_fmaf(fexp(0.5f * MV[zrow * LDM + nz + d]), ev[e], MV[zrow * LDM + d]);
+                img_put<CT, 16>(img, zrow, d, z);
+                if (store) Z[d] = to_ct<CT>(z);
+            }
+        }
+        if (tid < 16) img_put<CT, 16>(img, tid, nz, 1.0f);
+    }
+    lds_barrier();
+    AVAE_STAMP_EP(6)
+    if (wave < 2) {
+        f32x4 tacc[1][2] = {{{0.f, 0.f, 0.f, 0.f}, {0.f, 0.f, 0.f, 0.f}}};
+#pragma unroll
+        for (int sl = 0; sl < TSL; ++sl)
+            if (TSL == 2 || sl < t_sl) {
+                const u32x4 ta = *reinterpret_cast<const u32x4*>(img + (sl >> 1) * (16 * kTileBytesK) + fr * kTileBytesK + (((fq + 4 * (sl & 1)) ^ ((fr >> 1) & 7)) << 4));
+                mma<CT>(tb[sl][0], ta, tacc[0][0]);
+                mma<CT>(tb[sl][1], ta, tacc[0][1]);
+            }
+        regep_store<CT, 1, 2>(tacc, reinterpret_cast<CT*>(w.tail_out), w.tail_ldo, w.M, w.tail_n, m0 + fr, t_c0, lane,
+            [&](int, int, int, float v) { return act_fwd_t<ACT>(v); });
+    }
+    AVAE_STAMP(4)
+    AVAE_STAMP_FLUSH()
+}
+void launch_small_head(int compute_dtype, int act, int rows, const LaunchArgs& args, int grid_x, int grid_y, int lds_bytes, hipStream_t s,
                        unsigned long long* stamps, int launch_id) {
     const dim3 grid(grid_x, grid_y), block(kThreads);
-#define K_HEAD_B(A) k_small_head<__bf16, A>
-#define K_HEAD_F(A) k_small_head<float, A>
+#define K_HEAD_B(A) rows == 16 ? k_small_head16<__bf16, A> : k_small_head<__bf16, A>
+#define K_HEAD_F(A) rows == 16 ? k_small_head16<float, A> : k_small_head<float, A>
     if (compute_dtype == AVAE_BF16) {
         switch (act) {
             case AVAE_ACT_RELU: AVAE_LAUNCH((K_HEAD_B(AVAE_ACT_RELU)), grid, block, lds_bytes, s, args, stamps, launch_id); break;
@@ -1700,11 +1952,11 @@
 #undef K_HEAD_B
 #undef K_HEAD_F
 }
-void launch_small_latb(int compute_dtype, int act, const LaunchArgs& args, int grid_x, int grid_y, int lds_bytes, DevState* st, hipStream_t s,
+void launch_small_latb(int compute_dtype, int act, int rows, const LaunchArgs& args, int grid_x, int grid_y, int lds_bytes, DevState* st, hipStream_t s,
                        unsigned long long* stamps, int launch_id) {
     const dim3 grid(grid_x, grid_y), block(kThreads);
-#define K_LATB_B(A) k_small_latb<__bf16, A>
-#define K_LATB_F(A) k_small_latb<float, A>
+#define K_LATB_B(A) rows == 16 ? k_small_latb16<__bf16, A> : k_small_latb<__bf16, A>
+#define K_LATB_F(A) rows == 16 ? k_small_latb16<float, A> : k_small_latb<float, A>
     if (compute_dtype == AVAE_BF16) {
         switch (act) {
             case AVAE_ACT_RELU: AVAE_LAUNCH((K_LATB_B(AVAE_ACT_RELU)), grid, block, lds_bytes, s, args, st, stamps, launch_id); break;
@@ -1726,7 +1978,7 @@
 #undef K_LATB_F
 }
 
-template <typename CT, bool ADAM>
+template <typename CT, bool ADAM, bool STORE_G = true, bool COMPACT = false>
 __global__ void __launch_bounds__(kThreads) k_small_tn(const TnLaunchArgs args, unsigned long long* stamps, int launch_id) {
     constexpr int BM = 64, RING = 4, ES = (int)sizeof(CT), EPR = kTileBytesK / ES, NCH = 4;
     constexpr int kStage = 2 * BM * kTileBytesK;
@@ -1737,18 +1989,52 @@
     AVAE_STAMP(0)
     const int part = blockIdx.x & 7, idx = blockIdx.x >> 3;
     int entry = blockIdx.y, t_piece = -1;
-    if (args.xcd_pieces) {
-        const TnPiece* row = args.pieces[part];
-        int e = 0, lo = 0;
-#pragma unroll
-        for (int i = 0; i < kTnPieces; ++i) { const int ce = row[i].cum_end; if (idx >= ce) { e = i + 1; lo = ce; } }
-        if (e >= kTnPieces) return;
-        entry = row[e].item; t_piece = row[e].tile_off + idx - lo;
-    }
-    const TnItem w = args.items[entry];
-    asm volatile("" :: "s"(w.A), "s"(w.B), "s"(w.out), "s"(w.lda), "s"(w.ldb), "s"(w.K), "s"(w.ld0), "s"(w.tile_off));
+    TnItem w;
+    const DevState* st_ptr = nullptr;
+    if constexpr (COMPACT) {
+        unsigned long long q[kTnPieces][4];
+#pragma unroll
+        for (int i = 0; i < kTnPieces; ++i)
+#pragma unroll
+            for (int k = 0; k < 4; ++k) q[i][k] = args.desc[part][i].q[k];
+        st_ptr = args.st;
+        const int k_all = args.tn_k;
+        asm volatile("" :: "s"(st_ptr), "s"(k_all));
+#pragma unroll
+        for (int i = 0; i < kTnPieces; ++i) asm volatile("" :: "s"(q[i][0]), "s"(q[i][1]), "s"(q[i][2]), "s"(q[i][3]));
+        unsigned long long d0 = q[0][0], d1 = q[0][1], d2 = q[0][2], d3 = q[0][3];
+        int lo = 0;
+#pragma unroll
+        for (int i = 1; i < kTnPieces; ++i) {
+            const int ce = (int)((q[i - 1][3] >> 32) & 0xffffu);
+            const bool past = idx >= ce;
+            d0 = past ? q[i][0] : d0; d1 = past ? q[i][1] : d1; d2 = past ? q[i][2] : d2; d3 = past ? q[i][3] : d3;
+            lo = past ? ce : lo;
+        }
+        if (idx >= (int)((q[kTnPieces - 1][3] >> 32) & 0xffffu)) return;
+        w.A = reinterpret_cast<const void*>(d0); w.B = reinterpret_cast<const void*>(d1);
+        w.lda = (int)(unsigned)d2; w.ldb = (int)(unsigned)(d2 >> 32);
+        w.tiles_n = (int)(d3 & 0xffffu); w.K = k_all;
+        t_piece = (int)((d3 >> 16) & 0xffffu) + idx - lo;
+        entry = (int)(d3 >> 48);
+        const TnTail tl = args.tails[entry];
+        w.out = tl.out; w.W = tl.W; w.Wt = tl.Wt; w.M = tl.M; w.N = tl.N; w.ld0 = tl.ld0; w.ldw = tl.ldw; w.ldt = tl.ldt;
+        w.tile_off = 0; w.tile_cnt = 0;
+    } else {
+        if (args.xcd_pieces) {
+            const TnPiece* row = args.pieces[part];
+            int e = 0, lo = 0;
+#pragma unroll
+            for (int i = 0; i < kTnPieces; ++i) { const int ce = row[i].cum_end; if (idx >= ce) { e = i + 1; lo = ce; } }
+            if (e >= kTnPieces) return;
+            entry = row[e].item; t_piece = row[e].tile_off + idx - lo;
+        }
+        w = args.items[entry];
+        asm volatile("" :: "s"(w.A), "s"(w.B), "s"(w.out), "s"(w.lda), "s"(w.ldb), "s"(w.K), "s"(w.ld0), "s"(w.tile_off));
+        st_ptr = args.st;
+    }
     float lr_t = 0.f;
-    if constexpr (ADAM) lr_t = args.st->lr_t;
+    if constexpr (ADAM) lr_t = st_ptr->lr_t;
     int t;
     if (t_piece >= 0) {
         t = t_piece;
@@ -1873,7 +2159,7 @@
         }
         const bool full = m0 + BM <= w.M && n0 + BM <= w.N;
         auto store_group = [&](int k, float* gp, CT* wp) {
-            store4<float>(gp, g[k]);
+            if constexpr (STORE_G) store4<float>(gp, g[k]);
             store4<float>(gp + args.d_theta, th[k]); store4<float>(gp + args.d_m, m[k]); store4<float>(gp + args.d_v, v[k]);
             store4<CT>(wp, th[k]);
         };
@@ -1895,7 +2181,8 @@
                 } else if (grow < w.M && nv > 0) {
 #pragma unroll
                     for (int e = 0; e < 3; ++e) if (e < nv) {
-                        gp[e] = g[k][e]; gp[args.d_theta + e] = th[k][e]; gp[args.d_m + e] = m[k][e]; gp[args.d_v + e] = v[k][e]; wp[e] = to_ct<CT>(th[k][e]);
+                        if constexpr (STORE_G) gp[e] = g[k][e];
+                        gp[args.d_theta + e] = th[k][e]; gp[args.d_m + e] = m[k][e]; gp[args.d_v + e] = v[k][e]; wp[e] = to_ct<CT>(th[k][e]);
                     }
                     asm volatile("; partial quad" ::: "memory");
                 }
@@ -1920,11 +2207,23 @@
 void launch_small_tn(int compute_dtype, const TnLaunchArgs& args, int grid_x, int grid_y, hipStream_t s, unsigned long long* stamps, int launch_id) {
     const dim3 grid(grid_x, grid_y), block(kThreads);
     const int lds_bytes = 4 * 2 * 64 * kTileBytesK;
+    if (args.xcd_pieces == 2) {
+        if (compute_dtype == AVAE_BF16) {
+            if (args.adam == 2) AVAE_LAUNCH((k_small_tn<__bf16, true, false, true>), grid, block, lds_bytes, s, args, stamps, launch_id);
+            else AVAE_LAUNCH((k_small_tn<__bf16, true, true, true>), grid, block, lds_bytes, s, args, stamps, launch_id);
+        } else {
+            if (args.adam == 2) AVAE_LAUNCH((k_small_tn<float, true, false, true>), grid, block, lds_bytes, s, args, stamps, launch_id);
+            else AVAE_LAUNCH((k_small_tn<float, true, true, true>), grid, block, lds_bytes, s, args, stamps, launch_id);
+        }
+        return;
+    }
     if (compute_dtype == AVAE_BF16) {
-        if (args.adam) AVAE_LAUNCH((k_small_tn<__bf16, true>), grid, block, lds_bytes, s, args, stamps, launch_id);
+        if (args.adam == 2) AVAE_LAUNCH((k_small_tn<__bf16, true, false>), grid, block, lds_bytes, s, args, stamps, launch_id);
+        else if (args.adam) AVAE_LAUNCH((k_small_tn<__bf16, true>), grid, block, lds_bytes, s, args, stamps, launch_id);
         else AVAE_LAUNCH((k_small_tn<__bf16, false>), grid, block, lds_bytes, s, args, stamps, launch_id);
     } else {
-        if (args.adam) AVAE_LAUNCH((k_small_tn<float, true>), grid, block, lds_bytes, s, args, stamps, launch_id);
+        if (args.adam == 2) AVAE_LAUNCH((k_small_tn<float, true, false>), grid, block, lds_bytes, s, args, stamps, launch_id);
+        else if (args.adam) AVAE_LAUNCH((k_small_tn<float, true>), grid, block, lds_bytes, s, args, stamps, launch_id);
         else AVAE_LAUNCH((k_small_tn<float, false>), grid, block, lds_bytes, s, args, stamps, launch_id);
     }
 }
```

Result: faster. 4.920 million (median of 6 runs) (+3.7%).
